# zenithfang/supervised_dispnet

Hardware: AMD Instinct MI355X
Metric: images/sec fwd+bwd Disp_vgg_BN 128x416 b32 @1/2/4/8 GPU (higher is better)
Workload: dtype f32 (Winograd forward / input gradient / weight gradient form each f32 product from three exact bf16 pieces per operand on the bf16 matrix cores, six partial products, f32 accumulate; error vs fp64 at or below the f32 matrix instruction's)

## Files before the change

### include/dispnet_hip.h

```cpp
#ifndef DISPNET_HIP_H_
#define DISPNET_HIP_H_

#include <stddef.h>
#include <stdint.h>

#ifdef __cplusplus
extern "C" {
#endif

typedef void* dn_stream_t;

enum dn_status {
  DN_OK = 0,
  DN_ERR_BAD_ARG = -1,
  DN_ERR_UNSUPPORTED = -2,
  DN_ERR_WORKSPACE = -3,
  DN_ERR_LAUNCH = -4
};

void dn_reload_knobs(void);
int dn_version(void);
const char* dn_last_error(void);
const char* dn_last_kernel(void);
int dn_device_arch_ok(void);
// ... 14 lines not shown
  DN_CONVT_FWD = 2,
  DN_CONVT_DGRAD = 3
};

typedef struct dn_operand {
  const float* data;
  int32_t C;
  int32_t up_shift;
  int64_t stride_n, stride_h, stride_w, stride_c;
  const float* scale;
  const float* shift;
} dn_operand;

typedef struct dn_result {
  float* data;
  int32_t C;
  int32_t accumulate;
  int64_t stride_n, stride_h, stride_w;
} dn_result;

typedef struct dn_conv_desc {
  int32_t kind;
  int32_t N;
  int32_t IH, IW;
  int32_t OH, OW;
  int32_t R, S, stride, pad;
  int32_t n_in;
  dn_operand in[DN_MAX_OPERANDS];
  int32_t n_out;
  dn_result out[DN_MAX_OPERANDS];
  const float* w_packed;
  const float* bias;
  int32_t act;
  float act_p0, act_p1;
  float* bn_partial;
  int32_t pad_mode;
  int32_t compute;
  int32_t dilation;
  const float* bnb_y;
  const float* bnb_scale;
  const float* bnb_shift;
  const float* bnb_mean;
  const float* bnb_invstd;
  float* bnb_partial;
  void* splitk_ws;
  int64_t splitk_ws_bytes;
  float* recip_out;
  const float* bnf_gamma;
  const float* bnf_beta;
  float* bnf_running_mean;
  float* bnf_running_var;
  int64_t* bnf_num_batches_tracked;
  float bnf_momentum, bnf_eps;
  float* bnf_mean;
  float* bnf_invstd;
  float* bnf_scale;
  float* bnf_shift;
  float* bnb_dgamma;
  float* bnb_dbeta;
} dn_conv_desc;

enum { DN_COMPUTE_DEFAULT = 0, DN_COMPUTE_BF16 = 1, DN_COMPUTE_F32X3 = 2, DN_COMPUTE_F32 = 3 };

int64_t dn_conv_packed_weight_elems(const dn_conv_desc* d);
int dn_conv_pack_weights(const dn_conv_desc* d, const float* w, float* w_packed, dn_stream_t stream);
int64_t dn_pack_entry_bytes(void);
int dn_pack_entry_fill(const dn_conv_desc* d, const float* w, float* w_packed, void* entry_host);
int dn_pack_many(const void* entries_dev, int32_t n_direct, int32_t n_wino, int32_t n_wino_bf16, int32_t n_wino_x3, dn_stream_t stream);
int32_t dn_conv_weight_layout(const dn_conv_desc* d);
int32_t dn_conv_bn_partial_rows(const dn_conv_desc* d);
int64_t dn_conv_splitk_workspace_bytes(const dn_conv_desc* d);
int32_t dn_conv_fwd_folds_bn_finalize(const dn_conv_desc* d);
int32_t dn_conv_dgrad_folds_bn_sums(const dn_conv_desc* d);
int32_t dn_conv_dgrad_fuses_bn_sums(const dn_conv_desc* d);
int32_t dn_conv_fwd_fuses_reciprocal(const dn_conv_desc* d);
int dn_conv2d_fwd(const dn_conv_desc* d, dn_stream_t stream);
int dn_conv2d_dgrad(const dn_conv_desc* d, dn_stream_t stream);
int dn_convT2d_fwd(const dn_conv_desc* d, dn_stream_t stream);
int dn_convT2d_dgrad(const dn_conv_desc* d, dn_stream_t stream);

size_t dn_conv_wgrad_workspace_bytes(const dn_conv_desc* fwd);
int dn_conv2d_wgrad(const dn_conv_desc* fwd, const float* dy, float* dw, void* workspace, size_t workspace_bytes,
                    dn_stream_t stream);

int dn_bn_finalize(const float* partial, int32_t rows, int32_t C, int64_t count, const float* conv_bias,
                   const float* gamma, const float* beta, float* running_mean, float* running_var, float momentum,
                   float eps, float* mean, float* invstd, float* scale, float* shift, int64_t* num_batches_tracked,
                   dn_stream_t stream);
int dn_bn_eval_affine(int32_t C, const float* gamma, const float* beta, const float* running_mean,
                      const float* running_var, float eps, float* scale, float* shift, dn_stream_t stream);
int dn_bn_relu_pool_fwd(const float* y, const float* scale, const float* shift, int32_t N, int32_t H, int32_t W,
                        int32_t C, float* pooled, uint8_t* idx, dn_stream_t stream);
int dn_bn_relu_pool_bwd(const float* dpooled, const uint8_t* idx, const float* y, const float* mean,
                        const float* invstd, int32_t N, int32_t H, int32_t W, int32_t C, float* dz, float* partial,
                        dn_stream_t stream);
int dn_maxpool2_bwd(const float* dpooled, const uint8_t* idx, int32_t N, int32_t H, int32_t W, int32_t C, float* dx, int32_t accumulate,
                    dn_stream_t stream);
int dn_bn_relu_bwd_reduce(float* da_dz, const float* y, const float* scale, const float* shift, const float* mean,
                          const float* invstd, int64_t rows, int32_t C, float* partial, dn_stream_t stream);
int dn_bn_bwd_apply(float* dz_dy, const float* y, const float* mean, const float* invstd, const float* gamma,
                    const float* partial, int32_t partial_rows, int32_t partial_stride, int32_t partial_offset, int64_t rows,
                    int32_t C, float* dgamma, float* dbeta, dn_stream_t stream);
int dn_bn_relu_bwd_sums(const float* da, const float* y, const float* scale, const float* shift, const float* mean, const float* invstd,
                        int64_t rows, int32_t C, float* partial, dn_stream_t stream);
int dn_bn_relu_pool_bwd_sums(const float* dpooled, const uint8_t* idx, const float* y, const float* mean, const float* invstd, int32_t N,
                             int32_t H, int32_t W, int32_t C, float* partial, dn_stream_t stream);
int dn_bn_bwd_apply_relu(float* da_dy, const float* y, const float* scale, const float* shift, const float* mean, const float* invstd,
                         const float* gamma, const float* partial, int32_t partial_rows, int32_t partial_stride, int32_t partial_offset,
                         int64_t rows, int32_t C, float* dgamma, float* dbeta, dn_stream_t stream);
int dn_bn_bwd_apply_pool(const float* dpooled, const uint8_t* idx, const float* y, const float* mean, const float* invstd, const float* gamma,
                         const float* partial, int32_t partial_rows, int32_t partial_stride, int32_t partial_offset, int32_t N, int32_t H,
                         int32_t W, int32_t C, float* dy, float* dgamma, float* dbeta, dn_stream_t stream);
int32_t dn_reduce_blocks(int64_t rows, int32_t C);

int dn_act_bwd_reduce_from(const float* g_in, float* g_out, const float* y_post, int32_t act, float p0, float p1, int64_t rows, int32_t C,
                           float* partial, dn_stream_t stream);
int dn_act_bwd_reduce(float* g, const float* y_post, int32_t act, float p0, float p1, int64_t rows, int32_t C,
                      float* partial, dn_stream_t stream);
int dn_colsum_finalize(const float* partial, int32_t rows, int32_t C, int32_t stride, int32_t offset, float* out,
                       dn_stream_t stream);
int dn_upsample2x_nearest_bwd(const float* dfull, int32_t N, int32_t h, int32_t w, float* dlow, int32_t accumulate,
                              dn_stream_t stream);
int dn_upsample2x_nearest_bwd_nhwc(const float* dfull, int32_t N, int32_t h, int32_t w, int32_t C, float* dlow, int32_t accumulate,
                                   dn_stream_t stream);
int dn_reflect_fold(const float* dxp, int32_t N, int32_t H, int32_t W, int32_t C, int32_t pad, float* dx, int32_t accumulate,
                    dn_stream_t stream);
int dn_bn_add_relu_fwd(const float* y, const float* scale, const float* shift, const float* r, const float* r_scale, const float* r_shift,
                       int64_t rows, int32_t C, float* out, dn_stream_t stream);
int dn_bn_add_relu_bwd(const float* gout, const float* out, const float* y, const float* mean, const float* invstd, const float* r,
                       const float* r_mean, const float* r_invstd, int64_t rows, int32_t C, float* dz_y, float* dr, int32_t dr_accumulate,
                       float* partial, dn_stream_t stream);
int32_t dn_maxpool3s2_out(int32_t H, int32_t ceil_mode);
int dn_maxpool3s2_fwd(const float* x, int32_t N, int32_t H, int32_t W, int32_t C, int32_t ceil_mode, float* out, uint8_t* idx, dn_stream_t stream);
int dn_maxpool3s2_bwd(const float* dout, const uint8_t* idx, int32_t N, int32_t H, int32_t W, int32_t C, int32_t ceil_mode, float* dx,
                      int32_t accumulate, dn_stream_t stream);
int dn_sub_div(const float* x, int64_t n, float sub, float div, float* out, dn_stream_t stream);
int dn_upsample2x_bilinear_fwd(const float* low, int32_t N, int32_t h, int32_t w, int32_t OH, int32_t OW, float* out,
                               dn_stream_t stream);
int dn_upsample2x_bilinear_bwd(const float* dout, int32_t N, int32_t h, int32_t w, int32_t OH, int32_t OW, float* dlow,
                               int32_t accumulate, dn_stream_t stream);
int32_t dn_bn_stats_rows(int64_t rows);
int dn_bn_stats_partial(const float* x, int64_t rows, int32_t C, float* partial, dn_stream_t stream);
int dn_bn_apply_fwd(const float* y, const float* scale, const float* shift, int64_t rows, int32_t C, float* out, dn_stream_t stream);
int dn_phase_bias_add(float* x, int32_t N, int32_t H2, int32_t W2, int32_t C, const float* bias4, dn_stream_t stream);
size_t dn_phase_colsum_workspace_bytes(int32_t C);
int dn_phase_colsum(const float* g, int32_t N, int32_t H, int32_t W, int32_t C, float* workspace, float* out4, dn_stream_t stream);
int dn_act_fwd(const float* x, int64_t n, int32_t act, float p0, float p1, float* out, dn_stream_t stream);
int dn_resize_bilinear_fwd(const float* in, int32_t N, int32_t IH, int32_t IW, int32_t OH, int32_t OW, int32_t align_corners, float* out,
                           dn_stream_t stream);
int dn_resize_bilinear_bwd(const float* dout, int32_t N, int32_t IH, int32_t IW, int32_t OH, int32_t OW, int32_t align_corners, float* din,
                           int32_t accumulate, dn_stream_t stream);
int dn_spatial_mean_fwd(const float* x, int32_t N, int64_t HW, int32_t C, float scale, float* out, dn_stream_t stream);
int dn_spatial_mean_bwd(const float* dout, int32_t N, int64_t HW, int32_t C, float scale, float* dx, dn_stream_t stream);
int dn_reciprocal_fwd(const float* x, float* y, int64_t n, dn_stream_t stream);
int dn_reciprocal_bwd(const float* dy, const float* y, float* dx, int64_t n, dn_stream_t stream);

enum dn_masked_loss_kind { DN_LOSS_L1 = 0, DN_LOSS_L2 = 1, DN_LOSS_BERHU = 2, DN_LOSS_SCALE_INV = 3 };
#define DN_LOSS_STATS 8
size_t dn_masked_loss_workspace_bytes(int32_t G, int64_t pixels);
int dn_masked_loss_fwd(const float* gt, const float* pred, int32_t G, int64_t pixels, float max_depth, int32_t kind, float weight,
                       int32_t accumulate, float* stats, void* workspace, size_t workspace_bytes, float* loss, dn_stream_t stream);
int dn_masked_loss_fwd_fused(const float* gt, const float* pred, int32_t G, int64_t pixels, float max_depth, int32_t kind, float weight,
                             int32_t accumulate, float* stats, void* workspace, size_t workspace_bytes, float* loss, int32_t* counter,
                             dn_stream_t stream);
int dn_masked_loss_stats(const float* gt, const float* pred, int32_t G, int64_t pixels, float max_depth, int32_t kind, int32_t pass,
                         float* stats, void* workspace, size_t workspace_bytes, dn_stream_t stream);
int dn_masked_loss_finalize(float* stats, int32_t G, int32_t kind, float weight, int32_t accumulate, float* loss, dn_stream_t stream);
int dn_masked_loss_bwd(const float* gt, const float* pred, const float* stats, const float* dloss, int32_t G, int64_t pixels,
                       float max_depth, int32_t kind, float weight, float* dpred, dn_stream_t stream);
int dn_pyramid_down2(const float* in, int32_t N, int32_t H, int32_t W, int32_t mode, float* out, dn_stream_t stream);
int dn_upsample_int_fwd(const float* low, int32_t N, int32_t h, int32_t w, int32_t scale, int32_t mode, float* out, dn_stream_t stream);
int dn_upsample_int_bwd(const float* dout, int32_t N, int32_t h, int32_t w, int32_t scale, int32_t mode, float* dlow, dn_stream_t stream);
int32_t dn_reduce1d_blocks(int64_t n);
int dn_explainability_fwd(const float* mask, int64_t n, float weight, int32_t accumulate, float* partial, float* loss, dn_stream_t stream);
int dn_explainability_bwd(const float* mask, const float* dloss, int64_t n, float* dmask, dn_stream_t stream);
int32_t dn_smooth_blocks(int32_t B, int32_t H, int32_t W);
int dn_smooth2_fwd(const float* map, int32_t B, int32_t H, int32_t W, float weight, float* partial, float* loss,
                   dn_stream_t stream);
int dn_smooth2_bwd(const float* map, const float* dloss, int32_t B, int32_t H, int32_t W, float weight, float* dmap,
                   dn_stream_t stream);
int dn_compute_errors(const float* gt, const float* pred, int32_t B, int32_t H, int32_t W, float max_depth, int32_t y1,
                      int32_t y2, int32_t x1, int32_t x2, int32_t median_scaling, float* scratch, float* out8,
                      dn_stream_t stream);

int dn_pose_proj_fwd(const float* pose, int64_t pose_stride_b, const float* K, const float* Kinv, int32_t B, int32_t rotation_mode,
                     float downscale, float* proj, float* kinv_scaled, dn_stream_t stream);
int32_t dn_warp_blocks(int32_t h, int32_t w);
int dn_pose_proj_bwd(const float* pose, int64_t pose_stride_b, const float* K, int32_t B, int32_t rotation_mode, float downscale,
                     const float* dproj_partial, int32_t nblk, float* dpose, int64_t dpose_stride_b, int32_t accumulate,
                     dn_stream_t stream);
int dn_inverse_warp_fwd(const float* img, const float* depth, const float* proj, const float* kinv, int32_t B, int32_t h, int32_t w,
                        int32_t padding_mode, int32_t align_corners, float* warped, dn_stream_t stream);
// ... 108 lines not shown
```

### supervised_dispnet_amd/_lib.py

```python
import ctypes as C
import os
import pathlib

_PKG = pathlib.Path(__file__).resolve().parent
LIB_PATH = pathlib.Path(os.environ.get("DISPNET_HIP_LIB", _PKG / "libdispnet_hip.so"))

EXPECTED_ABI = 21

DN_MAX_OPERANDS = 3
ACT_NONE, ACT_RELU, ACT_LEAKY, ACT_ELU, ACT_SIGMOID_AFFINE = 0, 1, 2, 3, 4
COMPUTE_DEFAULT, COMPUTE_BF16, COMPUTE_F32X3, COMPUTE_F32 = 0, 1, 2, 3
CONV_FWD, CONV_DGRAD, CONVT_FWD, CONVT_DGRAD = 0, 1, 2, 3
LOSS_L1, LOSS_L2, LOSS_BERHU, LOSS_SCALE_INV = 0, 1, 2, 3
LOSS_STATS = 8

_f32p = C.c_void_p


class Operand(C.Structure):
    _fields_ = [("data", _f32p), ("C", C.c_int32), ("up_shift", C.c_int32),
                ("stride_n", C.c_int64), ("stride_h", C.c_int64), ("stride_w", C.c_int64), ("stride_c", C.c_int64),
                ("scale", _f32p), ("shift", _f32p)]


class Result(C.Structure):
    _fields_ = [("data", _f32p), ("C", C.c_int32), ("accumulate", C.c_int32),
                ("stride_n", C.c_int64), ("stride_h", C.c_int64), ("stride_w", C.c_int64)]


class ConvDesc(C.Structure):
    _fields_ = [("kind", C.c_int32), ("N", C.c_int32), ("IH", C.c_int32), ("IW", C.c_int32), ("OH", C.c_int32),
                ("OW", C.c_int32), ("R", C.c_int32), ("S", C.c_int32), ("stride", C.c_int32), ("pad", C.c_int32),
                ("n_in", C.c_int32), ("in_", Operand * DN_MAX_OPERANDS),
                ("n_out", C.c_int32), ("out", Result * DN_MAX_OPERANDS),
                ("w_packed", _f32p), ("bias", _f32p), ("act", C.c_int32), ("act_p0", C.c_float), ("act_p1", C.c_float),
                ("bn_partial", _f32p), ("pad_mode", C.c_int32), ("compute", C.c_int32), ("dilation", C.c_int32),
                ("bnb_y", _f32p), ("bnb_scale", _f32p), ("bnb_shift", _f32p), ("bnb_mean", _f32p), ("bnb_invstd", _f32p), ("bnb_partial", _f32p),
                ("splitk_ws", _f32p), ("splitk_ws_bytes", C.c_int64), ("recip_out", _f32p),
                ("bnf_gamma", _f32p), ("bnf_beta", _f32p), ("bnf_running_mean", _f32p), ("bnf_running_var", _f32p),
                ("bnf_num_batches_tracked", C.c_void_p), ("bnf_momentum", C.c_float), ("bnf_eps", C.c_float),
                ("bnf_mean", _f32p), ("bnf_invstd", _f32p), ("bnf_scale", _f32p), ("bnf_shift", _f32p),
                ("bnb_dgamma", _f32p), ("bnb_dbeta", _f32p)]


_P = C.POINTER
_i32, _i64, _f, _d, _vp, _sz = C.c_int32, C.c_int64, C.c_float, C.c_double, C.c_void_p, C.c_size_t

SIGNATURES = {
    "dn_version": (C.c_int, []),
    "dn_reload_knobs": (None, []),
    "dn_last_error": (C.c_char_p, []),
    "dn_last_kernel": (C.c_char_p, []),
    "dn_device_arch_ok": (C.c_int, []),
    "dn_conv_packed_weight_elems": (_i64, [_P(ConvDesc)]),
    "dn_conv_pack_weights": (C.c_int, [_P(ConvDesc), _vp, _vp, _vp]),
    "dn_pack_entry_bytes": (_i64, []),
    "dn_pack_entry_fill": (C.c_int, [_P(ConvDesc), _vp, _vp, _vp]),
    "dn_pack_many": (C.c_int, [_vp, _i32, _i32, _i32, _i32, _vp]),
    "dn_conv_weight_layout": (_i32, [_P(ConvDesc)]),
    "dn_conv_bn_partial_rows": (_i32, [_P(ConvDesc)]),
    "dn_conv_dgrad_fuses_bn_sums": (_i32, [_P(ConvDesc)]),
    "dn_conv_fwd_fuses_reciprocal": (_i32, [_P(ConvDesc)]),
    "dn_conv_splitk_workspace_bytes": (_i64, [_P(ConvDesc)]),
    "dn_conv_fwd_folds_bn_finalize": (_i32, [_P(ConvDesc)]),
    "dn_conv_dgrad_folds_bn_sums": (_i32, [_P(ConvDesc)]),
    "dn_conv2d_fwd": (C.c_int, [_P(ConvDesc), _vp]),
    "dn_conv2d_dgrad": (C.c_int, [_P(ConvDesc), _vp]),
    "dn_convT2d_fwd": (C.c_int, [_P(ConvDesc), _vp]),
    "dn_convT2d_dgrad": (C.c_int, [_P(ConvDesc), _vp]),
    "dn_conv_wgrad_workspace_bytes": (_sz, [_P(ConvDesc)]),
    "dn_conv2d_wgrad": (C.c_int, [_P(ConvDesc), _vp, _vp, _vp, _sz, _vp]),
    "dn_bn_finalize": (C.c_int, [_vp, _i32, _i32, _i64, _vp, _vp, _vp, _vp, _vp, _f, _f, _vp, _vp, _vp, _vp, _vp, _vp]),
    "dn_bn_eval_affine": (C.c_int, [_i32, _vp, _vp, _vp, _vp, _f, _vp, _vp, _vp]),
    "dn_bn_relu_pool_fwd": (C.c_int, [_vp, _vp, _vp, _i32, _i32, _i32, _i32, _vp, _vp, _vp]),
    "dn_bn_relu_bwd_sums": (C.c_int, [_vp, _vp, _vp, _vp, _vp, _vp, _i64, _i32, _vp, _vp]),
    "dn_bn_relu_pool_bwd_sums": (C.c_int, [_vp, _vp, _vp, _vp, _vp, _i32, _i32, _i32, _i32, _vp, _vp]),
    "dn_bn_bwd_apply_relu": (C.c_int, [_vp, _vp, _vp, _vp, _vp, _vp, _vp, _vp, _i32, _i32, _i32, _i64, _i32, _vp, _vp, _vp]),
    "dn_bn_bwd_apply_pool": (C.c_int, [_vp, _vp, _vp, _vp, _vp, _vp, _vp, _i32, _i32, _i32, _i32, _i32, _i32, _i32, _vp, _vp, _vp, _vp]),
    "dn_maxpool2_bwd": (C.c_int, [_vp, _vp, _i32, _i32, _i32, _i32, _vp, _i32, _vp]),
    "dn_bn_relu_pool_bwd": (C.c_int, [_vp, _vp, _vp, _vp, _vp, _i32, _i32, _i32, _i32, _vp, _vp, _vp]),
    "dn_bn_relu_bwd_reduce": (C.c_int, [_vp, _vp, _vp, _vp, _vp, _vp, _i64, _i32, _vp, _vp]),
    "dn_bn_bwd_apply": (C.c_int, [_vp, _vp, _vp, _vp, _vp, _vp, _i32, _i32, _i32, _i64, _i32, _vp, _vp, _vp]),
    "dn_reduce_blocks": (_i32, [_i64, _i32]),
    "dn_act_bwd_reduce": (C.c_int, [_vp, _vp, _i32, _f, _f, _i64, _i32, _vp, _vp]),
    "dn_act_bwd_reduce_from": (C.c_int, [_vp, _vp, _vp, _i32, _f, _f, _i64, _i32, _vp, _vp]),
    "dn_colsum_finalize": (C.c_int, [_vp, _i32, _i32, _i32, _i32, _vp, _vp]),
    "dn_upsample2x_nearest_bwd": (C.c_int, [_vp, _i32, _i32, _i32, _vp, _i32, _vp]),
    "dn_upsample2x_nearest_bwd_nhwc": (C.c_int, [_vp, _i32, _i32, _i32, _i32, _vp, _i32, _vp]),
    "dn_reflect_fold": (C.c_int, [_vp, _i32, _i32, _i32, _i32, _i32, _vp, _i32, _vp]),
    "dn_bn_add_relu_fwd": (C.c_int, [_vp, _vp, _vp, _vp, _vp, _vp, _i64, _i32, _vp, _vp]),
    "dn_bn_add_relu_bwd": (C.c_int, [_vp, _vp, _vp, _vp, _vp, _vp, _vp, _vp, _i64, _i32, _vp, _vp, _i32, _vp, _vp]),
    "dn_maxpool3s2_out": (_i32, [_i32, _i32]),
    "dn_maxpool3s2_fwd": (C.c_int, [_vp, _i32, _i32, _i32, _i32, _i32, _vp, _vp, _vp]),
    "dn_maxpool3s2_bwd": (C.c_int, [_vp, _vp, _i32, _i32, _i32, _i32, _i32, _vp, _i32, _vp]),
    "dn_bn_stats_rows": (_i32, [_i64]),
    "dn_bn_stats_partial": (C.c_int, [_vp, _i64, _i32, _vp, _vp]),
    "dn_bn_apply_fwd": (C.c_int, [_vp, _vp, _vp, _i64, _i32, _vp, _vp]),
    "dn_act_fwd": (C.c_int, [_vp, _i64, _i32, _f, _f, _vp, _vp]),
    "dn_phase_bias_add": (C.c_int, [_vp, _i32, _i32, _i32, _i32, _vp, _vp]),
    "dn_phase_colsum_workspace_bytes": (_sz, [_i32]),
    "dn_phase_colsum": (C.c_int, [_vp, _i32, _i32, _i32, _i32, _vp, _vp, _vp]),
    "dn_resize_bilinear_fwd": (C.c_int, [_vp, _i32, _i32, _i32, _i32, _i32, _i32, _vp, _vp]),
    "dn_resize_bilinear_bwd": (C.c_int, [_vp, _i32, _i32, _i32, _i32, _i32, _i32, _vp, _i32, _vp]),
    "dn_sub_div": (C.c_int, [_vp, _i64, _f, _f, _vp, _vp]),
    "dn_spatial_mean_fwd": (C.c_int, [_vp, _i32, _i64, _i32, _f, _vp, _vp]),
    "dn_spatial_mean_bwd": (C.c_int, [_vp, _i32, _i64, _i32, _f, _vp, _vp]),
    "dn_upsample2x_bilinear_fwd": (C.c_int, [_vp, _i32, _i32, _i32, _i32, _i32, _vp, _vp]),
    "dn_upsample2x_bilinear_bwd": (C.c_int, [_vp, _i32, _i32, _i32, _i32, _i32, _vp, _i32, _vp]),
    "dn_reciprocal_fwd": (C.c_int, [_vp, _vp, _i64, _vp]),
    "dn_reciprocal_bwd": (C.c_int, [_vp, _vp, _vp, _i64, _vp]),
    "dn_masked_loss_workspace_bytes": (_sz, [_i32, _i64]),
    "dn_masked_loss_fwd": (C.c_int, [_vp, _vp, _i32, _i64, _f, _i32, _f, _i32, _vp, _vp, _sz, _vp, _vp]),
    "dn_masked_loss_fwd_fused": (C.c_int, [_vp, _vp, _i32, _i64, _f, _i32, _f, _i32, _vp, _vp, _sz, _vp, _vp, _vp]),
    "dn_masked_loss_stats": (C.c_int, [_vp, _vp, _i32, _i64, _f, _i32, _i32, _vp, _vp, _sz, _vp]),
    "dn_masked_loss_finalize": (C.c_int, [_vp, _i32, _i32, _f, _i32, _vp, _vp]),
    "dn_masked_loss_bwd": (C.c_int, [_vp, _vp, _vp, _vp, _i32, _i64, _f, _i32, _f, _vp, _vp]),
    "dn_pyramid_down2": (C.c_int, [_vp, _i32, _i32, _i32, _i32, _vp, _vp]),
    "dn_upsample_int_fwd": (C.c_int, [_vp, _i32, _i32, _i32, _i32, _i32, _vp, _vp]),
    "dn_upsample_int_bwd": (C.c_int, [_vp, _i32, _i32, _i32, _i32, _i32, _vp, _vp]),
    "dn_reduce1d_blocks": (_i32, [_i64]),
    "dn_explainability_fwd": (C.c_int, [_vp, _i64, _f, _i32, _vp, _vp, _vp]),
    "dn_explainability_bwd": (C.c_int, [_vp, _vp, _i64, _vp, _vp]),
    "dn_smooth_blocks": (_i32, [_i32, _i32, _i32]),
    "dn_smooth2_fwd": (C.c_int, [_vp, _i32, _i32, _i32, _f, _vp, _vp, _vp]),
    "dn_smooth2_bwd": (C.c_int, [_vp, _vp, _i32, _i32, _i32, _f, _vp, _vp]),
    "dn_compute_errors": (C.c_int, [_vp, _vp, _i32, _i32, _i32, _f, _i32, _i32, _i32, _i32, _i32, _vp, _vp, _vp]),
    "dn_pose_proj_fwd": (C.c_int, [_vp, _i64, _vp, _vp, _i32, _i32, _f, _vp, _vp, _vp]),
    "dn_warp_blocks": (_i32, [_i32, _i32]),
    "dn_pose_proj_bwd": (C.c_int, [_vp, _i64, _vp, _i32, _i32, _f, _vp, _i32, _vp, _i64, _i32, _vp]),
    "dn_inverse_warp_fwd": (C.c_int, [_vp, _vp, _vp, _vp, _i32, _i32, _i32, _i32, _i32, _vp, _vp]),
    "dn_inverse_warp_bwd": (C.c_int, [_vp, _vp, _vp, _vp, _i32, _i32, _i32, _i32, _i32, _vp, _vp, _i32, _vp, _vp]),
    "dn_photometric_fwd": (C.c_int, [_vp, _vp, _vp, _vp, _vp, _vp, _i64, _i32, _i32, _i32, _i32, _i32, _f, _i32, _vp, _vp, _vp]),
    "dn_photometric_bwd": (C.c_int, [_vp, _vp, _vp, _vp, _vp, _vp, _i64, _i32, _i32, _i32, _i32, _i32, _f, _vp, _vp, _i32, _vp, _vp,
                                     _i64, _vp]),
    "dn_area_down": (C.c_int, [_vp, _i64, _i32, _i32, _i32, _vp, _vp]),
    "dn_ssim_fwd": (C.c_int, [_vp, _vp, _i64, _i32, _i32, _vp, _vp]),
    "dn_ssim_bwd": (C.c_int, [_vp, _vp, _vp, _i64, _i32, _i32, _vp, _vp, _vp, _vp]),
    "dn_edge_smooth_blocks": (_i32, [_i32, _i32, _i32]),
    "dn_edge_smooth_fwd": (C.c_int, [_vp, _vp, _i32, _i32, _i32, _i32, _vp, _vp, _vp]),
    "dn_edge_smooth_bwd": (C.c_int, [_vp, _vp, _vp, _i32, _i32, _i32, _i32, _vp, _vp]),
    "dn_ordinal_fwd": (C.c_int, [_vp, _i64, _i64, _i64, _i32, _i64, _i32, _vp, _vp, _vp]),
    "dn_ordinal_bwd": (C.c_int, [_vp, _i64, _i64, _i64, _vp, _vp, _i32, _i64, _i32, _vp, _vp]),
    "dn_ordinal_loss_blocks": (_i32, [_i32, _i64]),
    "dn_ordinal_loss_fwd": (C.c_int, [_vp, _vp, _vp, _i32, _i64, _i32, _f, _vp, _vp, _vp, _vp]),
    "dn_ordinal_loss_finalize": (C.c_int, [_vp, _vp, _vp]),
    "dn_ordinal_loss_bwd": (C.c_int, [_vp, _vp, _vp, _vp, _vp, _i32, _i64, _i32, _f, _f, _vp, _vp]),
    "dn_ord_head_supported": (_i32, [_i32, _i64, _i32]),
    "dn_ord_head_bwd_blocks": (_i32, [_i32, _i64]),
    "dn_ord_head_fwd": (C.c_int, [_vp, _vp, _vp, _vp, _i32, _i64, _i32, _vp, _vp, _vp]),
    "dn_ord_head_bwd": (C.c_int, [_vp, _vp, _vp, _vp, _vp, _i32, _i64, _i32, _vp, _i32, _vp, _vp, _vp, _vp]),
    "dn_sid_labels": (C.c_int, [_vp, _i64, _f, _f, _vp, _vp]),
    "dn_sid_depth": (C.c_int, [_vp, _i64, _f, _f, _vp, _vp]),
    "dn_channel_scale": (C.c_int, [_vp, _vp, _i32, _i64, _i32, _vp, _vp]),
    "dn_adam_step": (C.c_int, [_vp, _vp, _vp, _vp, _i64, _d, _d, _d, _d, _d, _i32, _d, _vp]),
    "dn_adam_step_dev": (C.c_int, [_vp, _vp, _vp, _vp, _i64, _vp, _d, _d, _vp, _vp, _d, _vp]),
    "dn_adam_tick": (C.c_int, [_vp, _vp, _vp, _vp]),
    "dn_fill": (C.c_int, [_vp, _f, _i64, _vp]),
    "dn_copy": (C.c_int, [_vp, _vp, _i64, _vp]),
    "dn_tape_begin": (_vp, []),
    "dn_tape_end": (C.c_int, [_vp]),
# ... 89 lines not shown
```

### supervised_dispnet_amd/csrc/dn_conv.hip

```cpp
#include <atomic>
#include <stdlib.h>
#include <type_traits>
#include <utility>

#include "dn_device.h"

namespace dn {

constexpr int LDK = 36;

struct AGroup {
  f32x4 v;
  bool ok;
};

__device__ __forceinline__ AGroup gather4(const KOperand& S, int kl, int ntaps, const int* taps, int n, int by, int bx,
                                          bool rowvalid, int IH, int IW, int j_vec, int c_vec, int reflect) {
  AGroup r;
  r.v = f32x4{0.f, 0.f, 0.f, 0.f};
  r.ok = false;
  if (S.vec) {
    if (rowvalid && j_vec < ntaps) {
      int t = taps[j_vec];
      int iy = by + (int)(short)(t & 0xffff), ix = bx + (t >> 16);
// ... 2165 lines not shown
    }
  }
  if (rc != DN_OK) return rc;
  return launch_wgrad_reduce(p, dw, s);
}

static bool wgrad_split_plans(const dn_conv_desc* fwd, dn_conv_desc* d1, dn_conv_desc* d2, IgemmParams* p1, IgemmParams* p2, size_t* w1,
                              size_t* w2) {
  if (fwd->kind != DN_CONV_FWD || fwd->n_in < 2 || fwd->in[fwd->n_in - 1].C != 1) return false;
  *d1 = *fwd;
  d1->n_in = fwd->n_in - 1;
  *d2 = *fwd;
  d2->n_in = 1;
  d2->in[0] = fwd->in[fwd->n_in - 1];
  if (build_plan(d1, true, p1) != DN_OK || build_plan(d2, true, p2) != DN_OK) return false;
  int cin_total = 0;
  for (int i = 0; i < fwd->n_in; ++i) cin_total += fwd->in[i].C;
  if (wino_wgrad_eligible(d1, *p1)) {
    p1->dw_cin_total = cin_total;
    *w1 = (wino_wgrad_workspace_bytes(*p1) + 255) / 256 * 256;
  } else {
    return false;
  }
  p2->in[0].ch_off = cin_total - 1;
  p2->D1 = cin_total;
  choose_splits(p2);
  *w2 = generic_wgrad_workspace_bytes(*p2);
  return true;
}

static int tap_windows(const IgemmParams& p) {
  const int nt = p.ph[0].ntaps;
  if (nt <= 32 || p.reflect || p.nphases != 1 || knobs().no_tap_windows) return 1;
  return (nt + 31) / 32;
}

static void tap_window_plan(const IgemmParams& full, int w, int nw, IgemmParams* q) {
  *q = full;
  const int nt = full.ph[0].ntaps, per = (nt + nw - 1) / nw;
  const int t0 = w * per, t1 = t0 + per < nt ? t0 + per : nt;
  for (int t = t0; t < t1; ++t) {
    q->tdy[t - t0] = full.tdy[full.ph[0].tap0 + t];
    q->tdx[t - t0] = full.tdx[full.ph[0].tap0 + t];
    q->tr[t - t0] = full.tr[full.ph[0].tap0 + t];
    q->ts[t - t0] = full.ts[full.ph[0].tap0 + t];
  }
  q->ph[0].tap0 = 0;
  q->ph[0].ntaps = t1 - t0;
  int nch = 0;
  for (int i = 0; i < q->n_in; ++i) nch += (q->ph[0].ntaps * q->in[i].C + kChunk - 1) / kChunk;
  q->ph[0].nchunks = nch;
  q->uni32 = 1;
  q->wg_uniform = 1;
  for (int i = 0; i < q->n_in; ++i) {
    const KOperand& o = q->in[i];
    if (!o.small) q->uni32 = 0;
    if (!o.small || (!o.vec && o.scale != nullptr) || o.C >= 32768) q->wg_uniform = 0;
  }
}

struct WgradFamily {
  const char* name;
  bool (*eligible)(const dn_conv_desc* fwd, const IgemmParams& p);
  size_t (*workspace_bytes)(const dn_conv_desc* fwd, const IgemmParams& p);
  bool dy_aligned16;
  bool (*switched_off)();
  int (*launch)(const dn_conv_desc* fwd, IgemmParams& p, float* dw, hipStream_t s);
};
static const WgradFamily kWgradFamilies[] = {
    {"head", head_wgrad_eligible, [](const dn_conv_desc*, const IgemmParams& p) { return head_wgrad_workspace_bytes(p); }, false,
     [] { return knobs().no_direct; },
     [](const dn_conv_desc*, IgemmParams& p, float* dw, hipStream_t s) { return launch_head_wgrad(p, dw, p.ws, s); }},
    {"winograd", wino_wgrad_eligible, [](const dn_conv_desc*, const IgemmParams& p) { return wino_wgrad_workspace_bytes(p); }, false, nullptr,
     [](const dn_conv_desc*, IgemmParams& p, float* dw, hipStream_t s) { return launch_wino_wgrad(p, dw, s); }},
    {"lds3", lds3_wgrad_eligible, [](const dn_conv_desc*, const IgemmParams& p) { return lds3_wgrad_workspace_bytes(p); }, true, nullptr,
     launch_lds3_wgrad},
    {"lds3k", lds3k_wgrad_eligible, [](const dn_conv_desc*, const IgemmParams& p) { return lds3k_wgrad_workspace_bytes(p); }, true, nullptr,
     launch_lds3k_wgrad},
    {"stemk", stemk_wgrad_eligible, stemk_wgrad_workspace_bytes, true, nullptr, launch_stemk_wgrad},
    {"thin", thin_wgrad_eligible, [](const dn_conv_desc*, const IgemmParams& p) { return thin_wgrad_workspace_bytes(p); }, false, nullptr,
     [](const dn_conv_desc*, IgemmParams& p, float* dw, hipStream_t s) { return launch_thin_wgrad(p, dw, s); }},
};

extern "C" {

int64_t dn_pack_entry_bytes(void) { return (int64_t)sizeof(PackEntry); }

int dn_pack_entry_fill(const dn_conv_desc* d, const float* w, float* w_packed, void* entry_host) {
  DN_REQUIRE(d && w && w_packed && entry_host, DN_ERR_BAD_ARG, "dn_pack_entry_fill: null pointer");
  PackEntry* e = reinterpret_cast<PackEntry*>(entry_host);
  int rc = build_plan(d, false, &e->p);
  if (rc != DN_OK) return rc;
  e->w = w;
  e->wp = w_packed;
  const ConvFamily* f = conv_route(d, e->p);
  e->wino = f->weight_layout ? f->weight_layout(e->p) : 0;
  if (e->wino) {
    e->total = wino_packed_elems(e->p);
    e->NS = ((e->p.Ntot + 63) / 64 * 64) / 32;
  } else {
    e->total = direct_packed_elems(e->p);
    e->NS = 0;
  }
  return e->wino;
}

int dn_pack_many(const void* entries_dev, int32_t n_direct, int32_t n_wino, int32_t n_wino16, int32_t n_wino_x3, dn_stream_t stream) {
  DN_REQUIRE(entries_dev && n_direct >= 0 && n_wino >= 0 && n_wino16 >= 0 && n_wino_x3 >= 0, DN_ERR_BAD_ARG, "dn_pack_many: bad argument");
  const PackEntry* tab = reinterpret_cast<const PackEntry*>(entries_dev);
  hipStream_t s = as_stream(stream);
  if (n_direct > 0) {
    DN_LAUNCH(pack_weights_many_kernel, dim3(knobs().pack_blocks, n_direct), dim3(256), 0, s, tab);
    int rc = check_launch("pack_weights_many_kernel");
    if (rc != DN_OK) return rc;
  }
  if (n_wino > 0) {
    int rc = launch_wino_pack_many(tab, n_direct, n_wino, s);
    if (rc != DN_OK) return rc;
  }
  if (n_wino16 > 0) {
    int rc = launch_wino_pack16_many(tab, n_direct + n_wino, n_wino16, 1, s);
    if (rc != DN_OK) return rc;
  }
  if (n_wino_x3 > 0) return launch_wino_pack16_many(tab, n_direct + n_wino + n_wino16, n_wino_x3, 3, s);
  return DN_OK;
}

int dn_conv_pack_weights(const dn_conv_desc* d, const float* w, float* w_packed, dn_stream_t stream) {
  IgemmParams p;
  int rc = build_plan(d, false, &p);
  if (rc != DN_OK) return rc;
  DN_REQUIRE(w != nullptr && w_packed != nullptr, DN_ERR_BAD_ARG, "null weight pointer");
  const ConvFamily* f = conv_route(d, p);
  if (const int wl = f->weight_layout ? f->weight_layout(p) : 0)
    return wl == 1 ? launch_wino_pack(p, w, w_packed, as_stream(stream)) : launch_wino_pack16(p, w, w_packed, wl == 3 ? 3 : 1, as_stream(stream));
  const long long total = direct_packed_elems(p);
  if (total == 0) return DN_OK;
  int blocks = (int)((total + 255) / 256);
  if (blocks > 4096) blocks = 4096;
  DN_LAUNCH(pack_weights_kernel, dim3(blocks), dim3(256), 0, as_stream(stream), p, w, w_packed, total);
  return check_launch("pack_weights_kernel");
}

int dn_conv2d_fwd(const dn_conv_desc* d, dn_stream_t stream) { return run_conv(d, DN_CONV_FWD, stream); }
int dn_conv2d_dgrad(const dn_conv_desc* d, dn_stream_t stream) { return run_conv(d, DN_CONV_DGRAD, stream); }
int dn_convT2d_fwd(const dn_conv_desc* d, dn_stream_t stream) { return run_conv(d, DN_CONVT_FWD, stream); }
int dn_convT2d_dgrad(const dn_conv_desc* d, dn_stream_t stream) { return run_conv(d, DN_CONVT_DGRAD, stream); }

size_t dn_conv_wgrad_workspace_bytes(const dn_conv_desc* fwd) {
  IgemmParams p;
  if (build_plan(fwd, true, &p) != DN_OK) return 0;
  choose_splits(&p);
  size_t need = generic_wgrad_workspace_bytes(p);
  for (const WgradFamily& f : kWgradFamilies)
    if (f.eligible(fwd, p) && f.workspace_bytes(fwd, p) > need) need = f.workspace_bytes(fwd, p);
  {
    dn_conv_desc d1, d2;
    IgemmParams p1, p2;
    size_t w1 = 0, w2 = 0;
    if (wgrad_split_plans(fwd, &d1, &d2, &p1, &p2, &w1, &w2) && w1 + w2 > need) need = w1 + w2;
  }
  const int nw = tap_windows(p);
  for (int w = 0; w < nw && nw > 1; ++w) {
    IgemmParams q;
    tap_window_plan(p, w, nw, &q);
    choose_splits(&q);
    if (generic_wgrad_workspace_bytes(q) > need) need = generic_wgrad_workspace_bytes(q);
  }
  return need;
}

int dn_conv2d_wgrad(const dn_conv_desc* fwd, const float* dy, float* dw, void* workspace, size_t workspace_bytes,
                    dn_stream_t stream) {
  IgemmParams p;
  int rc = build_plan(fwd, true, &p);
  if (rc != DN_OK) return rc;
  DN_REQUIRE(dy != nullptr && dw != nullptr && workspace != nullptr, DN_ERR_BAD_ARG, "null pointer");
  const hipStream_t s = as_stream(stream);
  for (const WgradFamily& f : kWgradFamilies) {
    if (!f.eligible(fwd, p) || (f.switched_off && f.switched_off()) || workspace_bytes < f.workspace_bytes(fwd, p)) continue;
    if (f.dy_aligned16 && (reinterpret_cast<uintptr_t>(dy) & 15) != 0) continue;
    for (int i = 0; i < p.n_in; ++i) DN_REQUIRE(p.in[i].p != nullptr, DN_ERR_BAD_ARG, "operand %d has no data", i);
    p.g = dy;
    p.ws = reinterpret_cast<float*>(workspace);
    return f.launch(fwd, p, dw, s);
  }
  {
    dn_conv_desc d1, d2;
    IgemmParams p1, p2;
    size_t w1 = 0, w2 = 0;
    if (wgrad_split_plans(fwd, &d1, &d2, &p1, &p2, &w1, &w2) && workspace_bytes >= w1 + w2) {
      for (int i = 0; i < fwd->n_in; ++i) DN_REQUIRE(fwd->in[i].data != nullptr, DN_ERR_BAD_ARG, "operand %d has no data", i);
      if (wino_wgrad_eligible(&d1, p1)) {
        p1.g = dy;
        p1.ws = reinterpret_cast<float*>(workspace);
        rc = launch_wino_wgrad(p1, dw, s);
      } else {
        rc = generic_wgrad(&d1, p1, dy, dw, workspace, w1, s);
      }
      if (rc != DN_OK) return rc;
      return generic_wgrad(&d2, p2, dy, dw, reinterpret_cast<char*>(workspace) + w1, w2, s);
    }
  }
  if (const int nw = tap_windows(p); nw > 1 && fwd->kind == DN_CONV_FWD) {
    for (int w = 0; w < nw; ++w) {
      IgemmParams q;
      tap_window_plan(p, w, nw, &q);
      rc = generic_wgrad(fwd, q, dy, dw, workspace, workspace_bytes, s);
      if (rc != DN_OK) return rc;
    }
    return DN_OK;
  }
  return generic_wgrad(fwd, p, dy, dw, workspace, workspace_bytes, s);
}

}
```

### supervised_dispnet_amd/csrc/dn_device.h

```cpp
#pragma once
#include <type_traits>
#include <utility>

#include "dn_internal.h"

namespace dn {

typedef float f32x2 __attribute__((ext_vector_type(2)));
typedef float f32x4 __attribute__((ext_vector_type(4)));
typedef float f32x16 __attribute__((ext_vector_type(16)));
typedef __bf16 bf16x2 __attribute__((ext_vector_type(2)));
typedef __bf16 bf16x4 __attribute__((ext_vector_type(4)));
typedef __bf16 bf16x8 __attribute__((ext_vector_type(8)));
typedef int i32x2 __attribute__((ext_vector_type(2)));
typedef int i32x4 __attribute__((ext_vector_type(4)));
typedef unsigned u32x4 __attribute__((ext_vector_type(4)));

template <class F, int... I>
__device__ __forceinline__ void static_for_impl(F&& f, std::integer_sequence<int, I...>) {
  (f(std::integral_constant<int, I>{}), ...);
}
template <int N, class F>
__device__ __forceinline__ void static_for(F&& f) {
  static_for_impl(f, std::make_integer_sequence<int, N>{});
}

__device__ __forceinline__ float apply_act(float v, int act, float p0, float p1) {
  switch (act) {
    case DN_ACT_RELU: return v > 0.f ? v : 0.f;
    case DN_ACT_LEAKY: return v > 0.f ? v : v * p0;
    case DN_ACT_ELU: return v > 0.f ? v : (expf(v) - 1.f);
    case DN_ACT_SIGMOID_AFFINE: return p0 / (1.f + expf(-v)) + p1;
    default: return v;
  }
}

__device__ __forceinline__ f32x4 apply_act4(f32x4 v, int act, float p0, float p1) {
  f32x4 r = v;
  switch (act) {
    case DN_ACT_RELU:
#pragma unroll
      for (int e = 0; e < 4; ++e) r[e] = v[e] > 0.f ? v[e] : 0.f;
      break;
    case DN_ACT_LEAKY:
#pragma unroll
      for (int e = 0; e < 4; ++e) r[e] = v[e] > 0.f ? v[e] : v[e] * p0;
      break;
    case DN_ACT_ELU:
#pragma unroll
      for (int e = 0; e < 4; ++e) r[e] = v[e] > 0.f ? v[e] : (expf(v[e]) - 1.f);
      break;
    case DN_ACT_SIGMOID_AFFINE:
#pragma unroll
      for (int e = 0; e < 4; ++e) r[e] = p0 / (1.f + expf(-v[e])) + p1;
      break;
    default: break;
  }
  return r;
}

__device__ __forceinline__ void split3(const float (&v)[8], bf16x8& h, bf16x8& m, bf16x8& l) {
#pragma unroll
  for (int e = 0; e < 8; e += 2) {
    const f32x2 x = f32x2{v[e], v[e + 1]};
    const bf16x2 h2 = __builtin_convertvector(x, bf16x2);
    const f32x2 r = x - __builtin_convertvector(h2, f32x2);
    const bf16x2 m2 = __builtin_convertvector(r, bf16x2);
    const f32x2 q = r - __builtin_convertvector(m2, f32x2);
    const bf16x2 l2 = __builtin_convertvector(q, bf16x2);
    h[e] = h2[0]; h[e + 1] = h2[1];
    m[e] = m2[0]; m[e + 1] = m2[1];
    l[e] = l2[0]; l[e + 1] = l2[1];
  }
}

__device__ __forceinline__ void wino_split3(float x, __bf16* pc) {
  pc[0] = (__bf16)x;
  const float r1 = x - (float)pc[0];
  pc[1] = (__bf16)r1;
  pc[2] = (__bf16)(r1 - (float)pc[1]);
}

__device__ __forceinline__ float wave_sum(float v) {
#pragma unroll
  for (int o = 32; o > 0; o >>= 1) v += __shfl_xor(v, o);
  return v;
}

template <int ROT>
__device__ __forceinline__ float dpp_row_ror(float v) {
  return __builtin_bit_cast(float, __builtin_amdgcn_update_dpp(0, __builtin_bit_cast(int, v), 0x120 + ROT, 0xf, 0xf, false));
}
__device__ __forceinline__ float row16_sum(float v) {
  v += dpp_row_ror<8>(v);
  v += dpp_row_ror<4>(v);
  v += dpp_row_ror<2>(v);
  v += dpp_row_ror<1>(v);
  return v;
}

template <int VW> struct VecOf;
template <> struct VecOf<4> { typedef f32x4 type; };
template <> struct VecOf<2> { typedef f32x2 type; };

template <int VW>
__device__ __forceinline__ typename VecOf<VW>::type buffer_load_vec(__amdgpu_buffer_rsrc_t r, int voffset) {
  if constexpr (VW == 4) {
    const i32x4 v = __builtin_amdgcn_raw_buffer_load_b128(r, voffset, 0, 0);
    return __builtin_bit_cast(f32x4, v);
  } else {
    const i32x2 v = __builtin_amdgcn_raw_buffer_load_b64(r, voffset, 0, 0);
    return __builtin_bit_cast(f32x2, v);
  }
}

__device__ __forceinline__ unsigned fastdiv_dev(unsigned n, unsigned d, unsigned M, unsigned* rem) {
  unsigned q = __umulhi(n, M);
  unsigned r = n - q * d;
  const bool fix = r >= d;
  q += fix ? 1u : 0u;
  r -= fix ? d : 0u;
  *rem = r;
  return q;
}

__device__ __forceinline__ int reflect_idx(int v, int n) {
  const int m = n - 1;
  int a = v < 0 ? -v : v;
  a = m - a;
  a = a < 0 ? -a : a;
  return m - a;
}

__device__ __forceinline__ int select_operand(const IgemmParams& p, int ntaps, int kc, int* kc_local) {
  int s = 0;
#pragma unroll
  for (int i = 0; i < DN_MAX_OPERANDS - 1; ++i) {
    if (s == i && i < p.n_in - 1) {
      int nch = (ntaps * p.in[i].C + kChunk - 1) / kChunk;
      if (kc >= nch) {
        kc -= nch;
// ... 10 lines not shown
```

### supervised_dispnet_amd/csrc/dn_internal.h

```cpp
#pragma once
#include <hip/hip_runtime.h>
#include <hip/hip_ext.h>
#include <stdint.h>
#include <stdio.h>

#include <atomic>
#include <functional>
#include <tuple>
#include <type_traits>

#include "dispnet_hip.h"

namespace dn {

void set_error(const char* fmt, ...);
void set_last_kernel(const char* fmt, ...);
int check_launch(const char* what);

static inline hipStream_t as_stream(dn_stream_t s) { return reinterpret_cast<hipStream_t>(s); }

struct LaunchTape;
extern std::atomic<LaunchTape*> g_tape_rec;
void tape_push(LaunchTape* t, std::function<void(hipEvent_t)>&& op, const void* kernel, hipStream_t stream);

// ... 141 lines not shown
  float* recip_out;
  float* ks_ws;
  size_t ks_ws_bytes;
  int T, TH, TW;
  unsigned mTW, mTH;
  BnFinalizeArgs bnf;
  float *bnb_dgamma, *bnb_dbeta;
  int* fold_cnt;
  int fold_bn, fold_bnb;
  int nmajor;
};

static inline unsigned fastdiv_magic(unsigned d) { return d <= 1 ? 0xFFFFFFFFu : (unsigned)(0x100000000ull / d); }

int build_plan(const dn_conv_desc* d, bool for_wgrad, IgemmParams* p);

inline long long direct_packed_elems(const IgemmParams& p) {
  const KPhase& last = p.ph[p.nphases - 1];
  return last.w_off + (long long)p.Npad * last.nchunks * kChunk;
}

struct PackEntry {
  IgemmParams p;
  const float* w;
  float* wp;
  long long total;
  int wino;
  int NS;
};
int launch_wino_pack_many(const PackEntry* tab_dev, int first, int n, hipStream_t stream);
int launch_wino_pack16_many(const PackEntry* tab_dev, int first, int n, int pieces, hipStream_t stream);
int launch_wino_pack16(const IgemmParams& p, const float* w, float* wp, int pieces, hipStream_t stream);
long long wino_packed_floats(const IgemmParams& p, int layout);
int wino_layout(const IgemmParams& p);

struct ConvFamily {
  const char* name;
  bool (*eligible)(const dn_conv_desc* d, const IgemmParams& p);
  bool (*switched_off)();
  int (*launch)(const dn_conv_desc* d, IgemmParams& p, hipStream_t s);
  int (*weight_layout)(const IgemmParams& p);
  size_t (*splitk_workspace_bytes)(const IgemmParams& p);
  bool (*fuses_reciprocal)(const IgemmParams& p);
  bool (*takes_bn_sums)(const dn_conv_desc* d);
  bool (*folds_bn_finalize)(IgemmParams& p);
  bool (*folds_bn_sums)(IgemmParams& p);
};
const ConvFamily* conv_route(const dn_conv_desc* d, const IgemmParams& p);

bool head_fwd_eligible(const dn_conv_desc* d, const IgemmParams& p);
int launch_head_fwd(const IgemmParams& p, hipStream_t stream);
bool head_fwd_fuses_reciprocal(const IgemmParams& p);
bool head_dgrad_eligible(const dn_conv_desc* d, const IgemmParams& p);
int launch_head_dgrad(const IgemmParams& p, hipStream_t stream);
bool head_wgrad_eligible(const dn_conv_desc* fwd, const IgemmParams& p);
size_t head_wgrad_workspace_bytes(const IgemmParams& p);
int launch_head_wgrad(const IgemmParams& p, float* dw, float* workspace, hipStream_t stream);

bool wino_eligible(const dn_conv_desc* d, const IgemmParams& p);
long long wino_packed_elems(const IgemmParams& p);
int launch_wino_pack(const IgemmParams& p, const float* w, float* wp, hipStream_t stream);
int launch_wino_conv(IgemmParams& p, hipStream_t stream);
void wino_prepare(IgemmParams& p);
bool wino_folds_bn_finalize(const IgemmParams& p);
bool wino_folds_bn_sums(const IgemmParams& p);
int wino_splitk_choice(const IgemmParams& p);
size_t conv_x3_splitk_workspace_upper_bytes(const IgemmParams& p);
size_t wino_splitk_workspace_bytes(const IgemmParams& p);
bool wino_wgrad_eligible(const dn_conv_desc* fwd, const IgemmParams& p);
size_t wino_wgrad_workspace_bytes(const IgemmParams& p);
int launch_wino_wgrad(IgemmParams& p, float* dw, hipStream_t stream);

bool thin_wgrad_eligible(const dn_conv_desc* fwd, const IgemmParams& p);
size_t thin_wgrad_workspace_bytes(const IgemmParams& p);
int launch_thin_wgrad(IgemmParams& p, float* dw, hipStream_t stream);
bool thin_conv_eligible(const dn_conv_desc* d, const IgemmParams& p);
int launch_thin_conv(const IgemmParams& p, hipStream_t stream);

bool lds3_conv_eligible(const dn_conv_desc* d, const IgemmParams& p);
int launch_lds3_conv(const dn_conv_desc* d, const IgemmParams& p, hipStream_t stream);
bool lds3_wgrad_eligible(const dn_conv_desc* fwd, const IgemmParams& p);
size_t lds3_wgrad_workspace_bytes(const IgemmParams& p);
int launch_lds3_wgrad(const dn_conv_desc* fwd, IgemmParams& p, float* dw, hipStream_t stream);
bool lds3k_wgrad_eligible(const dn_conv_desc* fwd, const IgemmParams& p);
size_t lds3k_wgrad_workspace_bytes(const IgemmParams& p);
int launch_lds3k_wgrad(const dn_conv_desc* fwd, IgemmParams& p, float* dw, hipStream_t stream);
int launch_wgrad_reduce(const IgemmParams& p, float* dw, hipStream_t stream);
bool wgrad_x3_eligible(const IgemmParams& p);
int launch_wgrad_x3(const IgemmParams& p, hipStream_t stream);
bool lds3k_conv_eligible(const dn_conv_desc* d, const IgemmParams& p);
int launch_lds3k_conv(const dn_conv_desc* d, const IgemmParams& p, hipStream_t stream);
bool stem3_conv_eligible(const dn_conv_desc* d, const IgemmParams& p);
bool stemk_conv_eligible(const dn_conv_desc* d, const IgemmParams& p);
int launch_stemk_conv(const dn_conv_desc* d, const IgemmParams& p, hipStream_t stream);
bool stemk_wgrad_eligible(const dn_conv_desc* d, const IgemmParams& p);
size_t stemk_wgrad_workspace_bytes(const dn_conv_desc* d, const IgemmParams& p);
int launch_stemk_wgrad(const dn_conv_desc* d, IgemmParams& p, float* dw, hipStream_t stream);
int launch_stem3_conv(const IgemmParams& p, hipStream_t stream);

}
```

### supervised_dispnet_amd/csrc/dn_lds3_wgrad.hip

```cpp
#include <stdlib.h>

#include "dn_device.h"

namespace dn {

struct WgGeo {
  int tilesX, tilesY, ntiles, per_xcd;
  long long slab;
  int dbgmode;
  long long* dbg;
};

constexpr int WG_TH = 8, WG_TW = 32;
constexpr int WG_GSTR = 528;
constexpr int WG_GPIECE = 16 * WG_GSTR;
constexpr int WG_XROWB = 96;
constexpr int WG_XSTR = 10 * WG_XROWB + 16;
constexpr int WG_XPIECE = 16 * WG_XSTR;
constexpr int WG_DCOLS = 36;
constexpr int WG16_LDS = 3 * WG_GPIECE + 3 * WG_XPIECE + 10 * WG_DCOLS * 4;

template <bool HAS1, bool DBG = false>
__global__ void __launch_bounds__(256, 2) lds3_wgrad16_kernel(const IgemmParams p, const WgGeo geo) {
  extern __shared__ __align__(16) char lds[];
// ... 116 lines not shown
      const int r = 2 * wave + rr;
      bf16x8 a[3];
#pragma unroll
      for (int P = 0; P < 3; ++P) a[P] = *reinterpret_cast<const bf16x8*>(Gp + P * WG_GPIECE + j * WG_GSTR + (r * 32 + 8 * g) * 2);
#pragma unroll
      for (int ty = 0; ty < 3; ++ty) {
        const char* rowb = Xp + j * WG_XSTR + (r + ty) * WG_XROWB + (8 * g + 8) * 2;
        u32x4 c[3];
        unsigned lf[3], rt[3];
#pragma unroll
        for (int P = 0; P < 3; ++P) {
          c[P] = *reinterpret_cast<const u32x4*>(rowb + P * WG_XPIECE);
          lf[P] = *reinterpret_cast<const unsigned*>(rowb + P * WG_XPIECE - 4);
          rt[P] = *reinterpret_cast<const unsigned*>(rowb + P * WG_XPIECE + 16);
        }
        bf16x8 bm[3], bz[3], bp[3];
#pragma unroll
        for (int P = 0; P < 3; ++P) {
          const u32x4 m4 = u32x4{__builtin_amdgcn_alignbit(c[P][0], lf[P], 16), __builtin_amdgcn_alignbit(c[P][1], c[P][0], 16),
                                 __builtin_amdgcn_alignbit(c[P][2], c[P][1], 16), __builtin_amdgcn_alignbit(c[P][3], c[P][2], 16)};
          const u32x4 p4 = u32x4{__builtin_amdgcn_alignbit(c[P][1], c[P][0], 16), __builtin_amdgcn_alignbit(c[P][2], c[P][1], 16),
                                 __builtin_amdgcn_alignbit(c[P][3], c[P][2], 16), __builtin_amdgcn_alignbit(rt[P], c[P][3], 16)};
          bm[P] = __builtin_bit_cast(bf16x8, m4);
          bz[P] = __builtin_bit_cast(bf16x8, c[P]);
          bp[P] = __builtin_bit_cast(bf16x8, p4);
        }
#pragma unroll
        for (int q = 0; q < 6; ++q) {
          acc[3 * ty + 0] = __builtin_amdgcn_mfma_f32_16x16x32_bf16(a[AS[q]], bm[BS[q]], acc[3 * ty + 0], 0, 0, 0);
          acc[3 * ty + 1] = __builtin_amdgcn_mfma_f32_16x16x32_bf16(a[AS[q]], bz[BS[q]], acc[3 * ty + 1], 0, 0, 0);
          acc[3 * ty + 2] = __builtin_amdgcn_mfma_f32_16x16x32_bf16(a[AS[q]], bp[BS[q]], acc[3 * ty + 2], 0, 0, 0);
        }
      }
      if constexpr (HAS1) {
        float v[8];
#pragma unroll
        for (int e = 0; e < 8; ++e) {
          const float x = Dp[r * WG_DCOLS + 8 * g + e + doff];
          v[e] = j < 9 ? x : 0.f;
        }
        bf16x8 b[3];
        split3(v, b[0], b[1], b[2]);
#pragma unroll
        for (int q = 0; q < 6; ++q) acc[9] = __builtin_amdgcn_mfma_f32_16x16x32_bf16(a[AS[q]], b[BS[q]], acc[9], 0, 0, 0);
      }
    }
    stamp(4);
    __syncthreads();
    stamp(5);
  }
  if constexpr (DBG) {
    if (lane == 0) {
      long long* o = geo.dbg + ((size_t)blockIdx.x * 8 + wave) * 8;
      for (int k = 0; k < 6; ++k) o[k] = tk[k];
      o[6] = (band_hi - band_lo - local + nlocal - 1) / nlocal;
    }
  }

  f32x4* red = reinterpret_cast<f32x4*>(lds);
#pragma unroll
  for (int t = 0; t < NT; ++t) red[(wave * NT + t) * 64 + lane] = acc[t];
  __syncthreads();
  const int Kp = p.ph[0].nchunks * kChunk;
  const int kbase1 = ((9 * 16 + kChunk - 1) / kChunk) * kChunk;
  float* slab = p.ws + (long long)blockIdx.x * geo.slab;
  for (int it = tid; it < NT * 64; it += 256) {
    const int t = it >> 6, l = it & 63;
    const f32x4 s = (red[(0 * NT + t) * 64 + l] + red[(1 * NT + t) * 64 + l]) + (red[(2 * NT + t) * 64 + l] + red[(3 * NT + t) * 64 + l]);
    const int jj = l & 15, gg = l >> 4;
    const int k = t < 9 ? t * 16 + jj : kbase1 + jj;
    if (t < 9 || jj < 9) {
#pragma unroll
      for (int e = 0; e < 4; ++e) slab[(long long)(4 * gg + e) * Kp + k] = s[e];
    }
  }
}

constexpr int WS_GSTR = 272;
constexpr int WS_GPIECE = 64 * WS_GSTR;
constexpr int WS_ICOLS = 36;
constexpr int WS_IPLANE = 10 * WS_ICOLS;
constexpr int WGS_LDS = 3 * WS_GPIECE + 3 * WS_IPLANE * 4;

__global__ void __launch_bounds__(256, 2) lds3_wgrad_stem_kernel(const IgemmParams p, const WgGeo geo) {
  extern __shared__ __align__(16) char lds[];
  char* Gp = lds;
  float* Ip = reinterpret_cast<float*>(lds + 3 * WS_GPIECE);
  const int tid = threadIdx.x, lane = tid & 63, wave = tid >> 6;
  const int j = lane & 15, g = lane >> 4;
  const KOperand& S = p.in[0];
  const int C = S.C, K = 9 * C;
  const __amdgpu_buffer_rsrc_t rg = __builtin_amdgcn_make_buffer_rsrc(const_cast<float*>(p.g), 0, 0x80000000u, 0x00020000);
  const __amdgpu_buffer_rsrc_t rx = __builtin_amdgcn_make_buffer_rsrc(const_cast<float*>(S.p), 0, 0x80000000u, 0x00020000);

  f32x4 acc[4][2];
#pragma unroll
  for (int m = 0; m < 4; ++m)
#pragma unroll
    for (int nt = 0; nt < 2; ++nt) acc[m][nt] = f32x4{0.f, 0.f, 0.f, 0.f};
  int ioff[2];
  bool ilive[2];
#pragma unroll
  for (int nt = 0; nt < 2; ++nt) {
    const int col = 16 * nt + j;
    ilive[nt] = col < K;
    const int tap = ilive[nt] ? col / C : 0, ci = ilive[nt] ? col - tap * C : 0;
    ioff[nt] = ci * WS_IPLANE + (tap / 3) * WS_ICOLS + (tap % 3);
  }

  f32x4 vg[8];
  float vi[4];
  auto issue_g = [&](int t, int h) __attribute__((always_inline)) {
    const int txb = t % geo.tilesX, q1 = t / geo.tilesX;
    const int tyb = q1 % geo.tilesY, n = q1 / geo.tilesY;
    const int pxg = tid & 15, cq = tid >> 4, row = pxg >> 2, cgp = pxg & 3;
    const int gy = tyb * WG_TH + 4 * h + row;
#pragma unroll
    for (int i = 0; i < 8; ++i) {
      const int gx = txb * WG_TW + 8 * cgp + i;
      const bool ok = gy < p.GH && gx < p.GW;
      const int off = (((n * p.GH + gy) * p.GW + gx) * p.Ntot + 4 * cq) * 4;
      vg[i] = __builtin_bit_cast(f32x4, __builtin_amdgcn_raw_buffer_load_b128(rg, ok ? off : -1, 0, 0));
    }
  };
  auto issue_img = [&](int t) __attribute__((always_inline)) {
    const int txb = t % geo.tilesX, q1 = t / geo.tilesX;
    const int tyb = q1 % geo.tilesY, n = q1 / geo.tilesY;
#pragma unroll
    for (int r = 0; r < 4; ++r) {
      const int it = tid + 256 * r;
      const int c = it / 340, px = it - c * 340;
      const int row = px / 34, col = px - row * 34;
      const int iy = tyb * WG_TH - 1 + row, ix = txb * WG_TW - 1 + col;
      const bool ok = c < C && (unsigned)iy < (unsigned)p.IH && (unsigned)ix < (unsigned)p.IW;
      const int off = (n * (int)S.sn + iy * (int)S.sh + ix * (int)S.sw + c * (int)S.sc) * 4;
      vi[r] = __builtin_bit_cast(float, __builtin_amdgcn_raw_buffer_load_b32(rx, ok ? off : -1, 0, 0));
    }
  };
  auto store_g = [&]() __attribute__((always_inline)) {
    const int pxg = tid & 15, cq = tid >> 4;
#pragma unroll
    for (int e = 0; e < 4; ++e) {
      const float v[8] = {vg[0][e], vg[1][e], vg[2][e], vg[3][e], vg[4][e], vg[5][e], vg[6][e], vg[7][e]};
      bf16x8 h, m, l;
      split3(v, h, m, l);
      char* dst = Gp + (4 * cq + e) * WS_GSTR + pxg * 16;
      *reinterpret_cast<bf16x8*>(dst) = h;
      *reinterpret_cast<bf16x8*>(dst + WS_GPIECE) = m;
      *reinterpret_cast<bf16x8*>(dst + 2 * WS_GPIECE) = l;
    }
  };
  auto store_img = [&]() __attribute__((always_inline)) {
#pragma unroll
    for (int r = 0; r < 4; ++r) {
      const int it = tid + 256 * r;
      const int c = it / 340, px = it - c * 340;
      const int row = px / 34, col = px - row * 34;
      if (c < 3) Ip[c * WS_IPLANE + row * WS_ICOLS + col] = vi[r];
    }
  };

  const int xcd = (int)blockIdx.x & 7, local = (int)blockIdx.x >> 3, nlocal = (int)gridDim.x >> 3;
  const int band_lo = xcd * geo.per_xcd, band_hi = min(band_lo + geo.per_xcd, geo.ntiles);
  constexpr int AS[6] = {0, 0, 1, 0, 1, 2}, BS[6] = {2, 1, 1, 0, 0, 0};
  if (band_lo + local < band_hi) {
    issue_g(band_lo + local, 0);
    issue_img(band_lo + local);
  }
  for (int t = band_lo + local; t < band_hi; t += nlocal) {
#pragma unroll 1
    for (int h = 0; h < 2; ++h) {
      store_g();
      if (h == 0) store_img();
      __syncthreads();
      if (h == 0) issue_g(t, 1);
      else if (t + nlocal < band_hi) {
        issue_g(t + nlocal, 0);
        issue_img(t + nlocal);
      }
      const int r = 4 * h + wave;
      bf16x8 b[2][3];
#pragma unroll
      for (int nt = 0; nt < 2; ++nt) {
        float v[8];
#pragma unroll
        for (int e = 0; e < 8; ++e) {
          const float x = Ip[r * WS_ICOLS + 8 * g + e + ioff[nt]];
          v[e] = ilive[nt] ? x : 0.f;
        }
        split3(v, b[nt][0], b[nt][1], b[nt][2]);
      }
#pragma unroll
      for (int m = 0; m < 4; ++m) {
        bf16x8 a[3];
#pragma unroll
        for (int P = 0; P < 3; ++P) a[P] = *reinterpret_cast<const bf16x8*>(Gp + P * WS_GPIECE + (16 * m + j) * WS_GSTR + (wave * 32 + 8 * g) * 2);
#pragma unroll
        for (int q = 0; q < 6; ++q)
#pragma unroll
          for (int nt = 0; nt < 2; ++nt) acc[m][nt] = __builtin_amdgcn_mfma_f32_16x16x32_bf16(a[AS[q]], b[nt][BS[q]], acc[m][nt], 0, 0, 0);
      }
      __syncthreads();
    }
  }

  f32x4* red = reinterpret_cast<f32x4*>(lds);
#pragma unroll
  for (int m = 0; m < 4; ++m)
#pragma unroll
    for (int nt = 0; nt < 2; ++nt) red[((wave * 4 + m) * 2 + nt) * 64 + lane] = acc[m][nt];
  __syncthreads();
  const int Kp = p.ph[0].nchunks * kChunk;
  float* slab = p.ws + (long long)blockIdx.x * geo.slab;
  for (int it = tid; it < 8 * 64; it += 256) {
    const int mn = it >> 6, l = it & 63, m = mn >> 1, nt = mn & 1;
    const f32x4 s = (red[((0 * 4 + m) * 2 + nt) * 64 + l] + red[((1 * 4 + m) * 2 + nt) * 64 + l]) +
                    (red[((2 * 4 + m) * 2 + nt) * 64 + l] + red[((3 * 4 + m) * 2 + nt) * 64 + l]);
    const int jj = l & 15, gg = l >> 4, k = 16 * nt + jj;
    if (k < K) {
#pragma unroll
      for (int e = 0; e < 4; ++e) slab[(long long)(16 * m + 4 * gg + e) * Kp + k] = s[e];
    }
  }
}

static int lds3_wgrad_form(const dn_conv_desc* d, const IgemmParams& p) {
  if (knobs().no_lds3 || norm_compute(d->compute) != DN_COMPUTE_F32X3) return 0;
  if (d->kind != DN_CONV_FWD || d->R != 3 || d->S != 3 || d->stride != 1 || d->pad != 1 || d->pad_mode != 0 || d->dilation > 1) return 0;
  if (d->IH != d->OH || d->IW != d->OW) return 0;
  if ((long long)p.M * p.Ntot * 4 + 64 >= (1ll << 31) || (reinterpret_cast<uintptr_t>(p.g) & 15)) return 0;
  for (int t = 0; t < 9; ++t)
    if (p.tdy[t] != t / 3 - 1 || p.tdx[t] != t % 3 - 1) return 0;
  const KOperand& a = p.in[0];
  if (!a.small || a.scale != nullptr || a.up != 0) return 0;
  if (p.Ntot == 16 && a.C == 16 && a.vec) {
    if (p.n_in == 1) return 1;
    const KOperand& b = p.in[1];
    if (p.n_in == 2 && b.C == 1 && b.small && b.scale == nullptr) return 2;
    return 0;
  }
  if (p.Ntot == 64 && p.n_in == 1 && a.C >= 1 && a.C <= 3) return 3;
  return 0;
}

static int lds3_wgrad_blocks(const IgemmParams& p) {
  const int ntiles = p.N * ((p.GH + WG_TH - 1) / WG_TH) * ((p.GW + WG_TW - 1) / WG_TW);
  int blocks = ntiles < 512 ? ntiles : 512;
  return (blocks + 7) / 8 * 8;
}

bool lds3_wgrad_eligible(const dn_conv_desc* d, const IgemmParams& p) { return lds3_wgrad_form(d, p) != 0; }

size_t lds3_wgrad_workspace_bytes(const IgemmParams& p) {
  return (size_t)lds3_wgrad_blocks(p) * p.Npad * p.ph[0].nchunks * kChunk * sizeof(float);
}

int launch_lds3_wgrad(const dn_conv_desc* d, IgemmParams& p, float* dw, hipStream_t stream) {
  const int form = lds3_wgrad_form(d, p);
  WgGeo geo;
  geo.tilesX = (p.GW + WG_TW - 1) / WG_TW;
  geo.tilesY = (p.GH + WG_TH - 1) / WG_TH;
  geo.ntiles = p.N * geo.tilesX * geo.tilesY;
  geo.per_xcd = (geo.ntiles + 7) / 8;
  geo.slab = (long long)p.Npad * p.ph[0].nchunks * kChunk;
  geo.dbg = knobs().lds3_dbg ? reinterpret_cast<long long*>(knobs().wino_dbgptr) : nullptr;
  geo.dbgmode = knobs().lds3_dbg;
  const int blocks = lds3_wgrad_blocks(p);
  hipError_t e = hipSuccess;
  if (geo.dbg != nullptr && form == 2) {
    e = hipFuncSetAttribute(reinterpret_cast<const void*>(lds3_wgrad16_kernel<true, true>), hipFuncAttributeMaxDynamicSharedMemorySize, WG16_LDS);
    if (e == hipSuccess) DN_LAUNCH((lds3_wgrad16_kernel<true, true>), dim3(blocks), dim3(256), (size_t)WG16_LDS, stream, p, geo);
    set_last_kernel("dn::lds3_wgrad16_kernel<true>");
  } else if (form == 3) {
    e = hipFuncSetAttribute(reinterpret_cast<const void*>(lds3_wgrad_stem_kernel), hipFuncAttributeMaxDynamicSharedMemorySize, WGS_LDS);
    if (e == hipSuccess) DN_LAUNCH(lds3_wgrad_stem_kernel, dim3(blocks), dim3(256), (size_t)WGS_LDS, stream, p, geo);
    set_last_kernel("dn::lds3_wgrad_stem_kernel");
  } else if (form == 2) {
    e = hipFuncSetAttribute(reinterpret_cast<const void*>(lds3_wgrad16_kernel<true>), hipFuncAttributeMaxDynamicSharedMemorySize, WG16_LDS);
    if (e == hipSuccess) DN_LAUNCH(lds3_wgrad16_kernel<true>, dim3(blocks), dim3(256), (size_t)WG16_LDS, stream, p, geo);
    set_last_kernel("dn::lds3_wgrad16_kernel<true>");
  } else if (form == 1) {
    e = hipFuncSetAttribute(reinterpret_cast<const void*>(lds3_wgrad16_kernel<false>), hipFuncAttributeMaxDynamicSharedMemorySize, WG16_LDS);
    if (e == hipSuccess) DN_LAUNCH(lds3_wgrad16_kernel<false>, dim3(blocks), dim3(256), (size_t)WG16_LDS, stream, p, geo);
    set_last_kernel("dn::lds3_wgrad16_kernel<false>");
  } else {
    set_error("launch_lds3_wgrad: no form");
    return DN_ERR_UNSUPPORTED;
  }
  if (e != hipSuccess) {
    set_error("lds3 wgrad: hipFuncSetAttribute: %s", hipGetErrorString(e));
    return DN_ERR_LAUNCH;
  }
  int rc = check_launch("lds3_wgrad_kernel");
  if (rc != DN_OK) return rc;
  p.splits = blocks;
  return launch_wgrad_reduce(p, dw, stream);
}

}

namespace dn {

constexpr int WK_TH = 2;
constexpr int WK_GSTR = WK_TH * 32 * 2 + 16;
constexpr int WK_GPIECE = 32 * WK_GSTR;
constexpr int WK_XROWS = WK_TH + 2;
constexpr int WK_XSTR = WK_XROWS * WG_XROWB + 16;
constexpr int WK_NCI = 96;
constexpr int WK_XPIECE = WK_NCI * WK_XSTR;
constexpr int WK_LDS = 3 * WK_GPIECE + 3 * WK_XPIECE + WK_XROWS * WG_DCOLS * 4;

template <bool HAS1, bool DBG = false>
__global__ void __launch_bounds__(512, 2) lds3k_wgrad_kernel(const IgemmParams p, const WgGeo geo, int c0) {
  extern __shared__ __align__(16) char lds[];
  char* Gp = lds;
  char* Xp = lds + 3 * WK_GPIECE;
  float* Dp = reinterpret_cast<float*>(lds + 3 * WK_GPIECE + 3 * WK_XPIECE);
  const int tid = threadIdx.x, lane = tid & 63, wave = tid >> 6;
  const int j = lane & 15, g = lane >> 4;
  const KOperand& S0 = p.in[0];
  const bool two = p.n_in - (HAS1 ? 1 : 0) == 2;
  const KOperand& S1 = p.in[two ? 1 : 0];
  const __amdgpu_buffer_rsrc_t rg = __builtin_amdgcn_make_buffer_rsrc(const_cast<float*>(p.g), 0, 0x80000000u, 0x00020000);
  const __amdgpu_buffer_rsrc_t r0 = __builtin_amdgcn_make_buffer_rsrc(const_cast<float*>(S0.p), 0, 0x80000000u, 0x00020000);
  const __amdgpu_buffer_rsrc_t r1 = __builtin_amdgcn_make_buffer_rsrc(const_cast<float*>(S1.p), 0, 0x80000000u, 0x00020000);
  const KOperand& SD = p.in[HAS1 ? p.n_in - 1 : 0];
  const __amdgpu_buffer_rsrc_t rd = __builtin_amdgcn_make_buffer_rsrc(const_cast<float*>(SD.p), 0, 0x80000000u, 0x00020000);

  const int nunits = wave < 2 ? 3 : 2;
  f32x4 acc[3][3][2];
#pragma unroll
  for (int u = 0; u < 3; ++u)
#pragma unroll
    for (int x = 0; x < 3; ++x)
#pragma unroll
      for (int m = 0; m < 2; ++m) acc[u][x][m] = f32x4{0.f, 0.f, 0.f, 0.f};
  f32x4 accd[2] = {f32x4{0.f, 0.f, 0.f, 0.f}, f32x4{0.f, 0.f, 0.f, 0.f}};
  const int dtap = j < 9 ? j : 0;
  const int doff = (dtap / 3) * WG_DCOLS + (dtap % 3);

  f32x4 va[8], vb[8];
  float dv = 0.f;
  const int nq0 = two ? c0 >> 2 : 24, n0jobs = 24 * nq0;
  auto decode = [&](int job, int& quad, int& rc, bool& second) __attribute__((always_inline)) {
    second = job >= n0jobs;
    const int jj = second ? job - n0jobs : job, nqh = (second ? 24 - nq0 : nq0) >> 2;
    const int rc_lo = jj & 3, q_lo = (jj >> 2) & 3, hi = jj >> 4;
    const int rc_hi = hi / nqh, q_hi = hi - rc_hi * nqh;
    rc = 4 * rc_hi + rc_lo;
    quad = (second ? nq0 : 0) + 4 * q_hi + q_lo;
  };
  int quadA, rcA, quadB, rcB;
  bool secA, secB;
  decode(tid, quadA, rcA, secA);
  decode(512 + (tid & 63), quadB, rcB, secB);
  const bool secAu = __builtin_amdgcn_readfirstlane((int)secA) != 0, secBu = __builtin_amdgcn_readfirstlane((int)secB) != 0;
  const int waveu = __builtin_amdgcn_readfirstlane(wave);
  const bool hasB = waveu == 2 || waveu == 3;
  const __amdgpu_buffer_rsrc_t rA = secAu ? r1 : r0;
// ... 312 lines not shown
```

### supervised_dispnet_amd/csrc/dn_plan.hip

```cpp
#include <stdarg.h>
#include <stdlib.h>
#include <string.h>

#include <atomic>
#include <mutex>

#include "dn_internal.h"

namespace dn {

static thread_local char g_err[512] = "";

void set_error(const char* fmt, ...) {
  va_list ap;
  va_start(ap, fmt);
  vsnprintf(g_err, sizeof(g_err), fmt, ap);
  va_end(ap);
}

static thread_local char g_kernel[160] = "";

void set_last_kernel(const char* fmt, ...) {
  va_list ap;
  va_start(ap, fmt);
// ... 272 lines not shown
          ph.ooy = py;
          ph.oox = px;
          for (int r = 0; r < d->R; ++r) {
            if (((py + pad - r * dil) % st + st) % st != 0) continue;
            for (int s = 0; s < d->S; ++s) {
              if (((px + pad - s * dil) % st + st) % st != 0) continue;
              DN_REQUIRE(nt < kMaxTaps, DN_ERR_UNSUPPORTED, "too many taps");
              p->tdy[nt] = (int8_t)floor_div(py + pad - r * dil, st);
              p->tdx[nt] = (int8_t)floor_div(px + pad - s * dil, st);
              p->tr[nt] = (int8_t)r;
              p->ts[nt] = (int8_t)s;
              ++nt;
            }
          }
          ph.ntaps = nt - ph.tap0;
        }
    }
    for (int i = 0; i < d->n_out; ++i) {
      KResult& r = p->out[i];
      r.p = d->out[i].data;
      r.C = d->out[i].C;
      r.accumulate = d->out[i].accumulate;
      r.sn = d->out[i].stride_n;
      r.sh = d->out[i].stride_h;
      r.sw = d->out[i].stride_w;
      r.n_begin = (i == 0) ? 0 : p->out[i - 1].n_begin + p->out[i - 1].C;
      r.linear = (p->nphases == 1 && r.sh == (long long)d->OW * r.sw && r.sn == (long long)d->OH * r.sh) ? 1 : 0;
    }
    DN_REQUIRE(d->bn_partial == nullptr || (d->n_out == 1 && p->nphases == 1), DN_ERR_UNSUPPORTED,
               "bn_partial needs a single un-phased result");
  }
  long long m = (long long)p->N * p->GH * p->GW;
  DN_REQUIRE(m > 0 && m < (1ll << 31), DN_ERR_UNSUPPORTED, "grid too large");
  p->M = (int)m;
  p->mGW = fastdiv_magic((unsigned)p->GW);
  p->mGH = fastdiv_magic((unsigned)p->GH);
  p->allvec = 1;
  p->uni32 = 1;
  p->any_affine = 0;
  for (int z = 0; z < p->nphases; ++z)
    if (p->ph[z].ntaps > 32) p->uni32 = 0;
  int n_fast = 0, n_uniform = 0;
  for (int i = 0; i < p->n_in; ++i) {
    const KOperand& o = p->in[i];
    if (o.scale != nullptr) p->any_affine = 1;
    p->in[i].small = offsets_fit_int32(p->in[i], p->N, p->IH, p->IW) && ((long long)p->N * (o.sn < 0 ? -o.sn : o.sn) + 16) * 4 < (1ll << 31) ? 1 : 0;
    if (!(p->in[i].vec && p->in[i].small)) p->allvec = 0;
    if (p->in[i].vec && p->in[i].small && o.up == 0 && (o.C % 32 == 0 || o.C == 4 || o.C == 8 || o.C == 16)) ++n_fast;
    if (p->in[i].vec && p->in[i].small && o.up == 0 && o.C % 32 == 0) ++n_uniform;
  }
  (void)n_fast;
  if (p->reflect) p->uni32 = 0;
  for (int i = 0; i < p->n_in; ++i)
    if (!p->in[i].small) p->uni32 = 0;
  p->wg_uniform = (!p->reflect && p->ph[0].ntaps <= 32) ? 1 : 0;
  for (int i = 0; i < p->n_in; ++i) {
    const KOperand& o = p->in[i];
    if (!o.small || (!o.vec && o.scale != nullptr) || o.C >= 32768) p->wg_uniform = 0;
  }
  (void)n_uniform;
  p->tile_store = false ? 0 : (false ? 1 : 2);
  p->compute = norm_compute(d->compute);
  p->BN = pick_bn(p->Ntot);
  p->Npad = ceil_div(p->Ntot, p->BN) * p->BN;
  long long woff = 0;
  for (int z = 0; z < p->nphases; ++z) {
    int nch = 0;
    for (int i = 0; i < p->n_in; ++i) nch += ceil_div(p->ph[z].ntaps * p->in[i].C, kChunk);
    p->ph[z].nchunks = nch;
    p->ph[z].w_off = woff;
    woff += (long long)p->Npad * nch * kChunk;
  }
  return DN_OK;
}

static const ConvFamily* plan_route(const dn_conv_desc* d, IgemmParams* p) {
  return build_plan(d, false, p) == DN_OK ? conv_route(d, *p) : nullptr;
}

}

extern "C" {

int dn_version(void) { return 21; }

void dn_reload_knobs(void) {
  std::lock_guard<std::mutex> lock(dn::g_knobs_mu);
  dn::read_knobs(&dn::g_knobs);
  dn::g_knobs_state.store(1, std::memory_order_release);
}

const char* dn_last_error(void) { return dn::g_err; }

const char* dn_last_kernel(void) { return dn::g_kernel; }

int dn_device_arch_ok(void) {
  int dev = 0;
  if (hipGetDevice(&dev) != hipSuccess) {
    dn::set_error("hipGetDevice failed (no HIP device?)");
    return DN_ERR_LAUNCH;
  }
  hipDeviceProp_t prop;
  if (hipGetDeviceProperties(&prop, dev) != hipSuccess) {
    dn::set_error("hipGetDeviceProperties failed");
    return DN_ERR_LAUNCH;
  }
  return strncmp(prop.gcnArchName, "gfx950", 6) == 0 ? 1 : 0;
}

int64_t dn_conv_packed_weight_elems(const dn_conv_desc* d) {
  dn::IgemmParams p;
  const dn::ConvFamily* f = dn::plan_route(d, &p);
  if (f == nullptr) return -1;
  return f->weight_layout ? dn::wino_packed_floats(p, f->weight_layout(p)) : dn::direct_packed_elems(p);
}

int32_t dn_conv_weight_layout(const dn_conv_desc* d) {
  dn::IgemmParams p;
  const dn::ConvFamily* f = dn::plan_route(d, &p);
  return f == nullptr ? -1 : (f->weight_layout ? f->weight_layout(p) : 0);
}

int32_t dn_conv_bn_partial_rows(const dn_conv_desc* d) {
  dn::IgemmParams p;
  if (dn::build_plan(d, false, &p) != DN_OK) return -1;
  return (p.M + 127) / 128;
}

int32_t dn_conv_fwd_fuses_reciprocal(const dn_conv_desc* d) {
  dn::IgemmParams p;
  const dn::ConvFamily* f = dn::plan_route(d, &p);
  return (f != nullptr && f->fuses_reciprocal && f->fuses_reciprocal(p)) ? 1 : 0;
}

int32_t dn_conv_dgrad_fuses_bn_sums(const dn_conv_desc* d) {
  dn::IgemmParams p;
  const dn::ConvFamily* f = dn::plan_route(d, &p);
  return f == nullptr ? -1 : ((f->takes_bn_sums && f->takes_bn_sums(d)) ? 1 : 0);
}

int32_t dn_conv_fwd_folds_bn_finalize(const dn_conv_desc* d) {
  dn::IgemmParams p;
  const dn::ConvFamily* f = dn::plan_route(d, &p);
  return f == nullptr ? -1 : ((f->folds_bn_finalize && f->folds_bn_finalize(p)) ? 1 : 0);
}

int32_t dn_conv_dgrad_folds_bn_sums(const dn_conv_desc* d) {
  dn::IgemmParams p;
  const dn::ConvFamily* f = dn::plan_route(d, &p);
  return (f != nullptr && f->takes_bn_sums && f->takes_bn_sums(d) && f->folds_bn_sums(p)) ? 1 : 0;
}

int64_t dn_conv_splitk_workspace_bytes(const dn_conv_desc* d) {
  dn::IgemmParams p;
  const dn::ConvFamily* f = dn::plan_route(d, &p);
  return f != nullptr ? (int64_t)f->splitk_workspace_bytes(p) : -1;
}

int dn_debug_conv_plan(const dn_conv_desc* d, int for_wgrad, int32_t* out, int cap) {
  dn::IgemmParams p;
  int rc = dn::build_plan(d, for_wgrad != 0, &p);
  if (rc != DN_OK) return rc;
  int n = 0;
  auto put = [&](long long v) {
    if (n < cap) out[n] = (int32_t)v;
    ++n;
  };
// ... 20 lines not shown
```

### supervised_dispnet_amd/csrc/dn_pointwise.hip

```cpp
#include "dn_device.h"
#include "dn_fold.h"

namespace dn {

constexpr int kThreads = 256;
constexpr int kMaxReduceBlocks = 4096;

static inline int ew_blocks(long long n_items) {
  long long b = (n_items + kThreads - 1) / kThreads;
  if (b > 4096) b = 4096;
  if (b < 1) b = 1;
  return (int)b;
}

static inline int reduce_blocks(long long rows, int C) {
  int V = (C % 4 == 0) ? 4 : 1;
  int groups = C / V;
  int tpr = 1;
  while (tpr < groups && tpr < kThreads) tpr <<= 1;
  int rpi = kThreads / tpr;
  const int rpt = 2;
  long long b = (rows + (long long)rpi * rpt - 1) / ((long long)rpi * rpt);
  const int cap = 1024 < kMaxReduceBlocks ? 1024 : kMaxReduceBlocks;
  if (b > cap) b = cap;
// ... 213 lines not shown
    pix /= PW;
    const int py = (int)(pix % PH), n = (int)(pix / PH);
    const uchar4 code = *reinterpret_cast<const uchar4*>(idx + i * 4);
    const f32x4 gv = *reinterpret_cast<const f32x4*>(dpooled + i * 4);
    float* base = dx + (((long long)n * H + 2 * py) * W + 2 * px) * C + g * 4;
#pragma unroll
    for (int q = 0; q < 4; ++q) {
      float* dst = base + ((long long)(q >> 1) * W + (q & 1)) * C;
      f32x4 o = accumulate ? *reinterpret_cast<const f32x4*>(dst) : f32x4{0.f, 0.f, 0.f, 0.f};
      if ((code.x & 3) == q) o[0] += gv[0];
      if ((code.y & 3) == q) o[1] += gv[1];
      if ((code.z & 3) == q) o[2] += gv[2];
      if ((code.w & 3) == q) o[3] += gv[3];
      *reinterpret_cast<f32x4*>(dst) = o;
    }
  }
}

struct PoolBwdOp {
  static constexpr int NACC = 2;
  const float* dpooled;
  const uint8_t* idx;
  const float* y;
  const float* mean;
  const float* invstd;
  float* dz;
  int PH, PW, H, W, C;
  template <int V>
  __device__ __forceinline__ void apply(long long row, int c0, float (&acc)[V][2]) const {
    const int px = (int)(row % PW);
    long long t = row / PW;
    const int py = (int)(t % PH), n = (int)(t / PH);
    const Vec<V> dp = ldv<V>(dpooled + row * C + c0);
    const Vec<V> mu = ldv<V>(mean + c0), is = ldv<V>(invstd + c0);
    const long long base = (((long long)n * H + 2 * py) * W + 2 * px) * C + c0;
    Vec<V> out[4];
#pragma unroll
    for (int q = 0; q < 4; ++q)
#pragma unroll
      for (int e = 0; e < V; ++e) out[q].v[e] = 0.f;
    unsigned codes = 0;
    if constexpr (V == 4) codes = *reinterpret_cast<const unsigned*>(idx + row * C + c0);
    Vec<V> yq[4];
#pragma unroll
    for (int q = 0; q < 4; ++q) yq[q] = ldv<V>(y + base + ((long long)(q >> 1) * W + (q & 1)) * C);
#pragma unroll
    for (int e = 0; e < V; ++e) {
      const int code = V == 4 ? (int)((codes >> (8 * e)) & 0xffu) : (int)idx[row * C + c0 + e];
      if (code & 4) {
        const int q = code & 3;
        const float g = dp.v[e];
        const float yv = q == 0 ? yq[0].v[e] : (q == 1 ? yq[1].v[e] : (q == 2 ? yq[2].v[e] : yq[3].v[e]));
#pragma unroll
        for (int qq = 0; qq < 4; ++qq)
          if (qq == q) out[qq].v[e] = g;
        acc[e][0] += g;
        acc[e][1] += g * (yv - mu.v[e]) * is.v[e];
      }
    }
    if (dz != nullptr) {
#pragma unroll
      for (int q = 0; q < 4; ++q) stv<V>(dz + base + ((long long)(q >> 1) * W + (q & 1)) * C, out[q]);
    }
  }
};

struct BnReluBwdOp {
  static constexpr int NACC = 2;
  int write;
  float* da_dz;
  const float* y;
  const float* scale;
  const float* shift;
  const float* mean;
  const float* invstd;
  int C;
  template <int V>
  __device__ __forceinline__ void apply(long long row, int c0, float (&acc)[V][2]) const {
    const long long o = row * C + c0;
    Vec<V> g = ldv<V>(da_dz + o);
    const Vec<V> yv = ldv<V>(y + o), sc = ldv<V>(scale + c0), sh = ldv<V>(shift + c0), mu = ldv<V>(mean + c0), is = ldv<V>(invstd + c0);
#pragma unroll
    for (int e = 0; e < V; ++e) {
      const float dz = (yv.v[e] * sc.v[e] + sh.v[e] > 0.f) ? g.v[e] : 0.f;
      g.v[e] = dz;
      acc[e][0] += dz;
      acc[e][1] += dz * (yv.v[e] - mu.v[e]) * is.v[e];
    }
    if (write) stv<V>(da_dz + o, g);
  }
};

struct ActBwdOp {
  static constexpr int NACC = 1;
  const float* src;
  float* g;
  const float* y_post;
  int act;
  float p0, p1;
  int C;
  template <int V>
  __device__ __forceinline__ void apply(long long row, int c0, float (&acc)[V][1]) const {
    const long long o = row * C + c0;
    Vec<V> gv = ldv<V>(src + o);
    if (act == DN_ACT_NONE) {
      if (src != g) stv<V>(g + o, gv);
    } else {
      const Vec<V> yv = ldv<V>(y_post + o);
#pragma unroll
      for (int e = 0; e < V; ++e) {
        const float yp = yv.v[e];
        float d = 1.f;
        if (act == DN_ACT_RELU) d = yp > 0.f ? 1.f : 0.f;
        else if (act == DN_ACT_LEAKY) d = yp > 0.f ? 1.f : p0;
        else if (act == DN_ACT_ELU) d = yp > 0.f ? 1.f : (yp + 1.f);
        else if (act == DN_ACT_SIGMOID_AFFINE) {
          const float sg = (yp - p1) / p0;
          d = p0 * sg * (1.f - sg);
        }
        gv.v[e] *= d;
      }
      stv<V>(g + o, gv);
    }
#pragma unroll
    for (int e = 0; e < V; ++e) acc[e][0] += gv.v[e];
  }
};

__global__ void __launch_bounds__(256) colsum_finalize_kernel(const float* __restrict__ partial, int rows, int C, int stride, int offset,
                                                              float* __restrict__ out) {
  const int lane = threadIdx.x & 63;
  const int c = blockIdx.x * 4 + (threadIdx.x >> 6);
  if (c >= C) return;
  double s = 0.0;
  for (int r = lane; r < rows; r += 64) s += (double)partial[((long long)r * C + c) * stride + offset];
#pragma unroll
  for (int o = 32; o > 0; o >>= 1) s += __shfl_xor(s, o);
  if (lane == 0) out[c] = (float)s;
}

__global__ void __launch_bounds__(256) colsum2_finalize_kernel(const float* __restrict__ partial, int rows, int C, int stride, int offset,
                                                               float* __restrict__ out0, float* __restrict__ out1) {
  const int c = blockIdx.x;
  double s0 = 0.0, s1 = 0.0;
#pragma unroll 4
  for (int r = threadIdx.x; r < rows; r += 256) {
    const float* q = partial + ((long long)r * C + c) * stride + offset;
    s0 += (double)q[0];
    s1 += (double)q[1];
  }
#pragma unroll
  for (int o = 32; o > 0; o >>= 1) {
    s0 += __shfl_xor(s0, o);
    s1 += __shfl_xor(s1, o);
  }
  __shared__ double red[2][4];
  if ((threadIdx.x & 63) == 0) {
    red[0][threadIdx.x >> 6] = s0;
    red[1][threadIdx.x >> 6] = s1;
  }
  __syncthreads();
  if (threadIdx.x == 0) {
    out0[c] = (float)((red[0][0] + red[0][1]) + (red[0][2] + red[0][3]));
    out1[c] = (float)((red[1][0] + red[1][1]) + (red[1][2] + red[1][3]));
  }
}

__device__ __forceinline__ float bn_bwd_value(float z, float yv, float mu, float is, float ga, float dg, float db, float inv_count) {
#pragma clang fp contract(off)
  const float xhat = (yv - mu) * is;
  float t = __builtin_fmaf(-db, inv_count, z);
  t = __builtin_fmaf(-(xhat * dg), inv_count, t);
  return (ga * is) * t;
}

__global__ void __launch_bounds__(kThreads) bn_bwd_apply_kernel(float* __restrict__ dz_dy, const float* __restrict__ y,
                                                                const float* __restrict__ mean, const float* __restrict__ invstd,
                                                                const float* __restrict__ gamma, const float* __restrict__ dgamma,
                                                                const float* __restrict__ dbeta, long long rows, int C, float inv_count) {
  const int G = C / 4;
  const long long total = rows * G;
  for (long long i = blockIdx.x * (long long)kThreads + threadIdx.x; i < total; i += (long long)gridDim.x * kThreads) {
    const int c = (int)(i % G) * 4;
    const long long o = i * 4;
    f32x4 dz = *reinterpret_cast<const f32x4*>(dz_dy + o);
    const f32x4 yv = *reinterpret_cast<const f32x4*>(y + o);
    const f32x4 mu = *reinterpret_cast<const f32x4*>(mean + c), is = *reinterpret_cast<const f32x4*>(invstd + c);
    const f32x4 ga = *reinterpret_cast<const f32x4*>(gamma + c), dg = *reinterpret_cast<const f32x4*>(dgamma + c),
                db = *reinterpret_cast<const f32x4*>(dbeta + c);
#pragma unroll
    for (int e = 0; e < 4; ++e) {
      dz[e] = bn_bwd_value(dz[e], yv[e], mu[e], is[e], ga[e], dg[e], db[e], inv_count);
    }
    *reinterpret_cast<f32x4*>(dz_dy + o) = dz;
  }
}

__global__ void __launch_bounds__(kThreads) bn_bwd_apply_relu_kernel(float* __restrict__ da_dy, const float* __restrict__ y,
                                                                     const float* __restrict__ scale, const float* __restrict__ shift,
                                                                     const float* __restrict__ mean, const float* __restrict__ invstd,
                                                                     const float* __restrict__ gamma, const float* __restrict__ dgamma,
                                                                     const float* __restrict__ dbeta, long long rows, int C, float inv_count) {
  const int G = C / 4;
  const long long total = rows * G;
  for (long long i = blockIdx.x * (long long)kThreads + threadIdx.x; i < total; i += (long long)gridDim.x * kThreads) {
    const int c = (int)(i % G) * 4;
    const long long o = i * 4;
    f32x4 dz = *reinterpret_cast<const f32x4*>(da_dy + o);
    const f32x4 yv = *reinterpret_cast<const f32x4*>(y + o);
    const f32x4 sc = *reinterpret_cast<const f32x4*>(scale + c), sh = *reinterpret_cast<const f32x4*>(shift + c);
    const f32x4 mu = *reinterpret_cast<const f32x4*>(mean + c), is = *reinterpret_cast<const f32x4*>(invstd + c);
    const f32x4 ga = *reinterpret_cast<const f32x4*>(gamma + c), dg = *reinterpret_cast<const f32x4*>(dgamma + c),
                db = *reinterpret_cast<const f32x4*>(dbeta + c);
#pragma unroll
    for (int e = 0; e < 4; ++e) {
      const float z = (yv[e] * sc[e] + sh[e] > 0.f) ? dz[e] : 0.f;
      dz[e] = bn_bwd_value(z, yv[e], mu[e], is[e], ga[e], dg[e], db[e], inv_count);
    }
    *reinterpret_cast<f32x4*>(da_dy + o) = dz;
  }
}

__global__ void __launch_bounds__(kThreads) bn_bwd_apply_relu_hoisted_kernel(float* __restrict__ da_dy, const float* __restrict__ y,
                                                                             const float* __restrict__ scale, const float* __restrict__ shift,
                                                                             const float* __restrict__ mean, const float* __restrict__ invstd,
                                                                             const float* __restrict__ gamma, const float* __restrict__ dgamma,
                                                                             const float* __restrict__ dbeta, long long rows, int C, float inv_count) {
  const int G = C / 4;
  const long long total = rows * G;
  const int c = (int)(threadIdx.x % (unsigned)G) * 4;
  const f32x4 sc = *reinterpret_cast<const f32x4*>(scale + c), sh = *reinterpret_cast<const f32x4*>(shift + c);
  const f32x4 mu = *reinterpret_cast<const f32x4*>(mean + c), is = *reinterpret_cast<const f32x4*>(invstd + c);
  const f32x4 ga = *reinterpret_cast<const f32x4*>(gamma + c), dg = *reinterpret_cast<const f32x4*>(dgamma + c),
              db = *reinterpret_cast<const f32x4*>(dbeta + c);
  const long long step = (long long)gridDim.x * kThreads;
  for (long long i0 = blockIdx.x * (long long)kThreads + threadIdx.x; i0 < total; i0 += 4 * step) {
    f32x4 dz[4], yv[4];
#pragma unroll
    for (int u = 0; u < 4; ++u) {
      const long long i = i0 + u * step;
      if (i < total) {
        dz[u] = __builtin_nontemporal_load(reinterpret_cast<const f32x4*>(da_dy + i * 4));
        yv[u] = __builtin_nontemporal_load(reinterpret_cast<const f32x4*>(y + i * 4));
      }
    }
#pragma unroll
    for (int u = 0; u < 4; ++u) {
      const long long i = i0 + u * step;
      if (i < total) {
#pragma unroll
        for (int e = 0; e < 4; ++e) {
          const float z = (yv[u][e] * sc[e] + sh[e] > 0.f) ? dz[u][e] : 0.f;
          dz[u][e] = bn_bwd_value(z, yv[u][e], mu[e], is[e], ga[e], dg[e], db[e], inv_count);
        }
        *reinterpret_cast<f32x4*>(da_dy + i * 4) = dz[u];
      }
    }
  }
}

__global__ void __launch_bounds__(kThreads) bn_bwd_apply_hoisted_kernel(float* __restrict__ dz_dy, const float* __restrict__ y,
                                                                        const float* __restrict__ mean, const float* __restrict__ invstd,
                                                                        const float* __restrict__ gamma, const float* __restrict__ dgamma,
                                                                        const float* __restrict__ dbeta, long long rows, int C, float inv_count) {
  const int G = C / 4;
  const long long total = rows * G;
  const long long first = blockIdx.x * (long long)kThreads + threadIdx.x;
  const int c = (int)(first % G) * 4;
  const f32x4 mu = *reinterpret_cast<const f32x4*>(mean + c), is = *reinterpret_cast<const f32x4*>(invstd + c);
  const f32x4 ga = *reinterpret_cast<const f32x4*>(gamma + c), dg = *reinterpret_cast<const f32x4*>(dgamma + c),
              db = *reinterpret_cast<const f32x4*>(dbeta + c);
  const long long step = (long long)gridDim.x * kThreads;
  for (long long i0 = first; i0 < total; i0 += 4 * step) {
    f32x4 dz[4], yv[4];
#pragma unroll
    for (int u = 0; u < 4; ++u) {
      const long long i = i0 + u * step;
      if (i < total) {
        dz[u] = __builtin_nontemporal_load(reinterpret_cast<const f32x4*>(dz_dy + i * 4));
        yv[u] = __builtin_nontemporal_load(reinterpret_cast<const f32x4*>(y + i * 4));
      }
    }
#pragma unroll
    for (int u = 0; u < 4; ++u) {
      const long long i = i0 + u * step;
      if (i < total) {
#pragma unroll
        for (int e = 0; e < 4; ++e) dz[u][e] = bn_bwd_value(dz[u][e], yv[u][e], mu[e], is[e], ga[e], dg[e], db[e], inv_count);
        *reinterpret_cast<f32x4*>(dz_dy + i * 4) = dz[u];
      }
    }
  }
}

__global__ void __launch_bounds__(kThreads) bn_bwd_apply_pool_kernel(const float* __restrict__ dpooled, const uint8_t* __restrict__ idx,
                                                                     const float* __restrict__ y, const float* __restrict__ mean,
                                                                     const float* __restrict__ invstd, const float* __restrict__ gamma,
                                                                     const float* __restrict__ dgamma, const float* __restrict__ dbeta, int N,
                                                                     int H, int W, int C, float inv_count, float* __restrict__ dy) {
  const int G = C / 4, PH = H / 2, PW = W / 2;
  const long long total = (long long)N * PH * PW * G;
  for (long long i = blockIdx.x * (long long)kThreads + threadIdx.x; i < total; i += (long long)gridDim.x * kThreads) {
    const int g = (int)(i % G);
    long long pix = i / G;
    const int px = (int)(pix % PW);
    pix /= PW;
    const int py = (int)(pix % PH), n = (int)(pix / PH);
    const int c = g * 4;
    const f32x4 dp = *reinterpret_cast<const f32x4*>(dpooled + i * 4);
    const uchar4 code = *reinterpret_cast<const uchar4*>(idx + i * 4);
    const int cd[4] = {code.x, code.y, code.z, code.w};
    const f32x4 mu = *reinterpret_cast<const f32x4*>(mean + c), is = *reinterpret_cast<const f32x4*>(invstd + c);
    const f32x4 ga = *reinterpret_cast<const f32x4*>(gamma + c), dg = *reinterpret_cast<const f32x4*>(dgamma + c),
                db = *reinterpret_cast<const f32x4*>(dbeta + c);
    const long long base = (((long long)n * H + 2 * py) * W + 2 * px) * C + c;
#pragma unroll
    for (int q = 0; q < 4; ++q) {
      const long long o = base + ((long long)(q >> 1) * W + (q & 1)) * C;
      const f32x4 yv = *reinterpret_cast<const f32x4*>(y + o);
      f32x4 out;
#pragma unroll
      for (int e = 0; e < 4; ++e) {
        const float z = ((cd[e] & 4) && (cd[e] & 3) == q) ? dp[e] : 0.f;
        out[e] = bn_bwd_value(z, yv[e], mu[e], is[e], ga[e], dg[e], db[e], inv_count);
      }
      *reinterpret_cast<f32x4*>(dy + o) = out;
    }
  }
}

__global__ void __launch_bounds__(kThreads) bn_add_relu_fwd_kernel(const float* __restrict__ y, const float* __restrict__ scale,
                                                                   const float* __restrict__ shift, const float* __restrict__ r,
                                                                   const float* __restrict__ r_scale, const float* __restrict__ r_shift,
                                                                   long long rows, int C, float* __restrict__ out) {
  const int G = C / 4;
// ... 387 lines not shown
  const long long total = (long long)N * (H / 2) * (W / 2) * (C / 4);
  DN_LAUNCH(bn_relu_pool_fwd_kernel, dim3(ew_blocks(total)), dim3(kThreads), 0, as_stream(stream), y, scale, shift, N, H, W, C,
                     pooled, idx);
  return check_launch("bn_relu_pool_fwd_kernel");
}

int dn_maxpool2_bwd(const float* dpooled, const uint8_t* idx, int32_t N, int32_t H, int32_t W, int32_t C, float* dx, int32_t accumulate,
                    dn_stream_t stream) {
  DN_REQUIRE(dpooled && idx && dx && N > 0, DN_ERR_BAD_ARG, "dn_maxpool2_bwd: bad argument");
  DN_REQUIRE(C % 4 == 0 && H % 2 == 0 && W % 2 == 0, DN_ERR_UNSUPPORTED, "dn_maxpool2_bwd: need C%%4==0 and even H,W");
  const long long total = (long long)N * (H / 2) * (W / 2) * (C / 4);
  DN_LAUNCH(maxpool2_bwd_kernel, dim3(ew_blocks(total)), dim3(kThreads), 0, as_stream(stream), dpooled, idx, N, H, W, C, dx, accumulate);
  return check_launch("maxpool2_bwd_kernel");
}

int dn_bn_relu_pool_bwd(const float* dpooled, const uint8_t* idx, const float* y, const float* mean, const float* invstd, int32_t N,
                        int32_t H, int32_t W, int32_t C, float* dz, float* partial, dn_stream_t stream) {
  DN_REQUIRE(dpooled && idx && y && mean && invstd && dz && partial, DN_ERR_BAD_ARG, "dn_bn_relu_pool_bwd: null pointer");
  DN_REQUIRE(C % 4 == 0 && H % 2 == 0 && W % 2 == 0, DN_ERR_UNSUPPORTED, "dn_bn_relu_pool_bwd: need C%%4==0 and even H,W");
  PoolBwdOp op{dpooled, idx, y, mean, invstd, dz, H / 2, W / 2, H, W, C};
  return launch_colreduce(op, (long long)N * (H / 2) * (W / 2), C, partial, as_stream(stream), "bn_relu_pool_bwd");
}

int dn_bn_relu_pool_bwd_sums(const float* dpooled, const uint8_t* idx, const float* y, const float* mean, const float* invstd, int32_t N,
                             int32_t H, int32_t W, int32_t C, float* partial, dn_stream_t stream) {
  DN_REQUIRE(dpooled && idx && y && mean && invstd && partial, DN_ERR_BAD_ARG, "dn_bn_relu_pool_bwd_sums: null pointer");
  DN_REQUIRE(C % 4 == 0 && H % 2 == 0 && W % 2 == 0, DN_ERR_UNSUPPORTED, "dn_bn_relu_pool_bwd_sums: need C%%4==0 and even H,W");
  PoolBwdOp op{dpooled, idx, y, mean, invstd, nullptr, H / 2, W / 2, H, W, C};
  return launch_colreduce(op, (long long)N * (H / 2) * (W / 2), C, partial, as_stream(stream), "bn_relu_pool_bwd_sums");
}

int dn_bn_relu_bwd_reduce(float* da_dz, const float* y, const float* scale, const float* shift, const float* mean, const float* invstd,
                          int64_t rows, int32_t C, float* partial, dn_stream_t stream) {
  DN_REQUIRE(da_dz && y && scale && shift && mean && invstd && partial && rows > 0 && C > 0, DN_ERR_BAD_ARG,
             "dn_bn_relu_bwd_reduce: bad argument");
  BnReluBwdOp op{1, da_dz, y, scale, shift, mean, invstd, C};
  return launch_colreduce(op, rows, C, partial, as_stream(stream), "bn_relu_bwd_reduce");
}

int dn_bn_relu_bwd_sums(const float* da, const float* y, const float* scale, const float* shift, const float* mean, const float* invstd,
                        int64_t rows, int32_t C, float* partial, dn_stream_t stream) {
  DN_REQUIRE(da && y && scale && shift && mean && invstd && partial && rows > 0 && C > 0, DN_ERR_BAD_ARG, "dn_bn_relu_bwd_sums: bad argument");
  BnReluBwdOp op{0, const_cast<float*>(da), y, scale, shift, mean, invstd, C};
  return launch_colreduce(op, rows, C, partial, as_stream(stream), "bn_relu_bwd_sums");
}

static void launch_colsum2(const float* partial, int32_t partial_rows, int32_t C, int32_t partial_stride, int32_t partial_offset, float* out0,
                           float* out1, hipStream_t s) {
  if (partial_rows <= kFoldMaxRows && (partial_stride & 1) == 0 && (partial_offset & 1) == 0 && (reinterpret_cast<uintptr_t>(partial) & 7) == 0)
    DN_LAUNCH(colsum2_sliced_kernel, dim3((C + 63) / 64), dim3(256), 0, s, partial, partial_rows, C, partial_stride, partial_offset, out0, out1);
  else
    DN_LAUNCH(colsum2_finalize_kernel, dim3(C), dim3(256), 0, s, partial, partial_rows, C, partial_stride, partial_offset, out0, out1);
}

static int bn_bwd_sums_to_params(const float* partial, int32_t partial_rows, int32_t partial_stride, int32_t partial_offset, int32_t C,
                                 float* dgamma, float* dbeta, hipStream_t s, const char* who) {
  DN_REQUIRE(dgamma && dbeta, DN_ERR_BAD_ARG, "%s: bad argument", who);
  DN_REQUIRE(C % 4 == 0, DN_ERR_UNSUPPORTED, "%s: need C%%4==0", who);
  if (partial == nullptr) return DN_OK;
  DN_REQUIRE(partial_rows > 0, DN_ERR_BAD_ARG, "%s: bad argument", who);
  DN_REQUIRE(partial_stride >= 2 && partial_offset >= 0 && partial_offset + 1 < partial_stride, DN_ERR_BAD_ARG, "%s: partial layout", who);
  launch_colsum2(partial, partial_rows, C, partial_stride, partial_offset, dbeta, dgamma, s);
  return DN_OK;
}

int dn_bn_bwd_apply_relu(float* da_dy, const float* y, const float* scale, const float* shift, const float* mean, const float* invstd,
                         const float* gamma, const float* partial, int32_t partial_rows, int32_t partial_stride, int32_t partial_offset,
                         int64_t rows, int32_t C, float* dgamma, float* dbeta, dn_stream_t stream) {
  DN_REQUIRE(da_dy && y && scale && shift && mean && invstd && gamma && rows > 0, DN_ERR_BAD_ARG, "dn_bn_bwd_apply_relu: bad argument");
  hipStream_t s = as_stream(stream);
  int rc = bn_bwd_sums_to_params(partial, partial_rows, partial_stride, partial_offset, C, dgamma, dbeta, s, "dn_bn_bwd_apply_relu");
  if (rc != DN_OK) return rc;
  const bool hoisted = C % 4 == 0 && kThreads % (C / 4) == 0;
  set_last_kernel(hoisted ? "dn::bn_bwd_apply_relu_hoisted_kernel" : "dn::bn_bwd_apply_relu_kernel");
  if (hoisted)
    DN_LAUNCH(bn_bwd_apply_relu_hoisted_kernel, dim3(ew_blocks((rows * (C / 4) + 3) / 4)), dim3(kThreads), 0, s, da_dy, y, scale, shift, mean,
              invstd, gamma, dgamma, dbeta, (long long)rows, C, (float)(1.0 / (double)rows));
  else
    DN_LAUNCH(bn_bwd_apply_relu_kernel, dim3(ew_blocks(rows * (C / 4))), dim3(kThreads), 0, s, da_dy, y, scale, shift, mean, invstd, gamma,
                     dgamma, dbeta, (long long)rows, C, (float)(1.0 / (double)rows));
  return check_launch("bn_bwd_apply_relu");
}

int dn_bn_bwd_apply_pool(const float* dpooled, const uint8_t* idx, const float* y, const float* mean, const float* invstd, const float* gamma,
                         const float* partial, int32_t partial_rows, int32_t partial_stride, int32_t partial_offset, int32_t N, int32_t H,
                         int32_t W, int32_t C, float* dy, float* dgamma, float* dbeta, dn_stream_t stream) {
  DN_REQUIRE(dpooled && idx && y && mean && invstd && gamma && dy && N > 0, DN_ERR_BAD_ARG, "dn_bn_bwd_apply_pool: bad argument");
  DN_REQUIRE(H % 2 == 0 && W % 2 == 0, DN_ERR_UNSUPPORTED, "dn_bn_bwd_apply_pool: need even H, W");
  hipStream_t s = as_stream(stream);
  int rc = bn_bwd_sums_to_params(partial, partial_rows, partial_stride, partial_offset, C, dgamma, dbeta, s, "dn_bn_bwd_apply_pool");
  if (rc != DN_OK) return rc;
  const long long total = (long long)N * (H / 2) * (W / 2) * (C / 4);
  DN_LAUNCH(bn_bwd_apply_pool_kernel, dim3(ew_blocks(total)), dim3(kThreads), 0, s, dpooled, idx, y, mean, invstd, gamma, dgamma, dbeta, N,
                     H, W, C, (float)(1.0 / ((double)N * H * W)), dy);
  return check_launch("bn_bwd_apply_pool");
}

int dn_bn_bwd_apply(float* dz_dy, const float* y, const float* mean, const float* invstd, const float* gamma, const float* partial,
                    int32_t partial_rows, int32_t partial_stride, int32_t partial_offset, int64_t rows, int32_t C, float* dgamma,
                    float* dbeta, dn_stream_t stream) {
  DN_REQUIRE(dz_dy && y && mean && invstd && gamma && partial && dgamma && dbeta && rows > 0, DN_ERR_BAD_ARG, "dn_bn_bwd_apply: bad argument");
  DN_REQUIRE(C % 4 == 0, DN_ERR_UNSUPPORTED, "dn_bn_bwd_apply: need C%%4==0");
  DN_REQUIRE(partial_stride >= 2 && partial_offset >= 0 && partial_offset + 1 < partial_stride, DN_ERR_BAD_ARG, "dn_bn_bwd_apply: partial layout");
  hipStream_t s = as_stream(stream);
  launch_colsum2(partial, partial_rows, C, partial_stride, partial_offset, dbeta, dgamma, s);
  const int G = C / 4;
  int blocks = ew_blocks((rows * (long long)G + 3) / 4);
  int ga = G, gb = kThreads;
  while (gb != 0) {
    const int t = ga % gb;
    ga = gb;
    gb = t;
  }
  const int per = G / ga;
  if (per <= 64) {
    blocks = (blocks + per - 1) / per * per;
    set_last_kernel("dn::bn_bwd_apply_hoisted_kernel");
    DN_LAUNCH(bn_bwd_apply_hoisted_kernel, dim3(blocks), dim3(kThreads), 0, s, dz_dy, y, mean, invstd, gamma, dgamma, dbeta, (long long)rows, C,
              (float)(1.0 / (double)rows));
  } else {
    set_last_kernel("dn::bn_bwd_apply_kernel");
    DN_LAUNCH(bn_bwd_apply_kernel, dim3(ew_blocks(rows * (C / 4))), dim3(kThreads), 0, s, dz_dy, y, mean, invstd, gamma, dgamma, dbeta,
              (long long)rows, C, (float)(1.0 / (double)rows));
  }
  return check_launch("bn_bwd_apply");
}

int dn_act_bwd_reduce(float* g, const float* y_post, int32_t act, float p0, float p1, int64_t rows, int32_t C, float* partial,
                      dn_stream_t stream) {
  DN_REQUIRE(g && partial && rows > 0 && C > 0 && (act == DN_ACT_NONE || y_post), DN_ERR_BAD_ARG, "dn_act_bwd_reduce: bad argument");
  ActBwdOp op{g, g, y_post, act, p0, p1, C};
  return launch_colreduce(op, rows, C, partial, as_stream(stream), "act_bwd_reduce");
}

int dn_act_bwd_reduce_from(const float* g_in, float* g_out, const float* y_post, int32_t act, float p0, float p1, int64_t rows, int32_t C,
                           float* partial, dn_stream_t stream) {
  DN_REQUIRE(g_in && g_out && partial && rows > 0 && C > 0 && (act == DN_ACT_NONE || y_post), DN_ERR_BAD_ARG, "dn_act_bwd_reduce_from: bad argument");
  ActBwdOp op{g_in, g_out, y_post, act, p0, p1, C};
  return launch_colreduce(op, rows, C, partial, as_stream(stream), "act_bwd_reduce_from");
}

int dn_colsum_finalize(const float* partial, int32_t rows, int32_t C, int32_t stride, int32_t offset, float* out, dn_stream_t stream) {
  DN_REQUIRE(partial && out && rows > 0 && C > 0 && stride > 0 && offset >= 0 && offset < stride, DN_ERR_BAD_ARG, "dn_colsum_finalize: bad argument");
  DN_LAUNCH(colsum_finalize_kernel, dim3((C + 3) / 4), dim3(256), 0, as_stream(stream), partial, rows, C, stride, offset, out);
  return check_launch("colsum_finalize_kernel");
}

int dn_upsample2x_nearest_bwd(const float* dfull, int32_t N, int32_t h, int32_t w, float* dlow, int32_t accumulate, dn_stream_t stream) {
  DN_REQUIRE(dfull && dlow && N > 0 && h > 0 && w > 0, DN_ERR_BAD_ARG, "dn_upsample2x_nearest_bwd: bad argument");
  DN_LAUNCH(upsample2x_nearest_bwd_kernel, dim3(ew_blocks((long long)N * h * w)), dim3(256), 0, as_stream(stream), dfull, N, h, w,
                     dlow, accumulate);
  return check_launch("upsample2x_nearest_bwd_kernel");
}

int dn_upsample2x_bilinear_fwd(const float* low, int32_t N, int32_t h, int32_t w, int32_t OH, int32_t OW, float* out, dn_stream_t stream) {
  DN_REQUIRE(low && out && N > 0 && OH <= 2 * h && OW <= 2 * w && OH > 0 && OW > 0, DN_ERR_BAD_ARG, "dn_upsample2x_bilinear_fwd: bad argument");
  DN_LAUNCH(upsample2x_bilinear_fwd_kernel, dim3(ew_blocks((long long)N * OH * OW)), dim3(256), 0, as_stream(stream), low, N, h, w,
                     OH, OW, out);
  return check_launch("upsample2x_bilinear_fwd_kernel");
}

int dn_upsample2x_bilinear_bwd(const float* dout, int32_t N, int32_t h, int32_t w, int32_t OH, int32_t OW, float* dlow, int32_t accumulate,
                               dn_stream_t stream) {
  DN_REQUIRE(dout && dlow && N > 0 && OH <= 2 * h && OW <= 2 * w && OH > 0 && OW > 0, DN_ERR_BAD_ARG, "dn_upsample2x_bilinear_bwd: bad argument");
  DN_LAUNCH(upsample2x_bilinear_bwd_kernel, dim3(ew_blocks((long long)N * h * w)), dim3(256), 0, as_stream(stream), dout, N, h, w,
                     OH, OW, dlow, accumulate);
// ... 143 lines not shown
```

### supervised_dispnet_amd/csrc/dn_wino_common.h

```cpp
#pragma once
#include "dn_device.h"
#include "dn_fold.h"

namespace dn {

constexpr int WBT = 64;
constexpr int WBN = 64;
constexpr int WKC = 16;
constexpr int WZLD = 72;

template <int MTW>
struct WinoCfg {
  static constexpr int BT = 32 * MTW;
  static constexpr int HALFB = BT * 16 + 32;
  static constexpr int POSB = 2 * HALFB;
  static constexpr int SUBB = 16 * POSB + 64;
  static constexpr int BUFB = 2 * SUBB;
  static constexpr size_t LDS = (size_t)2 * BUFB;
};

constexpr int W16_ROWB = 48;

template <int NK, int TSTEP, int NWAVES, int GROUPS>
__device__ __forceinline__ void wino_bn_bwd_sums(const IgemmParams& p, const f32x4 (&Y)[NK][2][2], int mb, int tg, int c4, int wave, int lane, int tid,
                                                 int n_first, float* red) {
  constexpr int BT = 32 * GROUPS;
  f32x4 s1[GROUPS], s2[GROUPS];
#pragma unroll
  for (int g = 0; g < GROUPS; ++g) s1[g] = s2[g] = f32x4{0.f, 0.f, 0.f, 0.f};
  if (n_first < p.Ntot) {
    const f32x4 sc = *reinterpret_cast<const f32x4*>(p.bnb_scale + n_first), sh = *reinterpret_cast<const f32x4*>(p.bnb_shift + n_first);
    const f32x4 mu = *reinterpret_cast<const f32x4*>(p.bnb_mean + n_first), is = *reinterpret_cast<const f32x4*>(p.bnb_invstd + n_first);
    const long long C = p.Ntot, rowB = (long long)p.OW * C;
#pragma unroll
    for (int k = 0; k < NK; ++k) {
      const int t = mb * BT + tg + TSTEP * k;
      if (t < p.T) {
        unsigned tx, ty;
        const unsigned r = fastdiv_dev((unsigned)t, (unsigned)p.TW, p.mTW, &tx);
        const int n = (int)fastdiv_dev(r, (unsigned)p.TH, p.mTH, &ty);
        const float* y00 = p.bnb_y + (((long long)n * p.OH + 2 * (int)ty) * p.OW + 2 * (int)tx) * C + n_first;
        const f32x4 yv[2][2] = {{*reinterpret_cast<const f32x4*>(y00), *reinterpret_cast<const f32x4*>(y00 + C)},
                                {*reinterpret_cast<const f32x4*>(y00 + rowB), *reinterpret_cast<const f32x4*>(y00 + rowB + C)}};
#pragma unroll
        for (int a = 0; a < 2; ++a)
#pragma unroll
          for (int b = 0; b < 2; ++b)
#pragma unroll
            for (int e = 0; e < 4; ++e) {
              const float yy = yv[a][b][e];
              const float dz = (yy * sc[e] + sh[e] > 0.f) ? Y[k][a][b][e] : 0.f;
              s1[(k * TSTEP) / 32][e] += dz;
              s2[(k * TSTEP) / 32][e] += dz * (yy - mu[e]) * is[e];
            }
      }
    }
  }
#pragma unroll
  for (int g = 0; g < GROUPS; ++g)
#pragma unroll
    for (int e = 0; e < 4; ++e) {
      s1[g][e] += __shfl_xor(s1[g][e], 16);
      s1[g][e] += __shfl_xor(s1[g][e], 32);
      s2[g][e] += __shfl_xor(s2[g][e], 16);
      s2[g][e] += __shfl_xor(s2[g][e], 32);
    }
  __syncthreads();
  if (lane < 16) {
#pragma unroll
    for (int g = 0; g < GROUPS; ++g) {
      *reinterpret_cast<f32x4*>(red + ((g * NWAVES + wave) * 2 + 0) * 64 + 4 * c4) = s1[g];
      *reinterpret_cast<f32x4*>(red + ((g * NWAVES + wave) * 2 + 1) * 64 + 4 * c4) = s2[g];
    }
  }
  __syncthreads();
  if (tid < 64 * GROUPS) {
    const int g = tid >> 6, col = tid & 63;
    float a1 = 0.f, a2 = 0.f;
#pragma unroll
    for (int w = 0; w < NWAVES; ++w) {
      a1 += red[((g * NWAVES + w) * 2 + 0) * 64 + col];
      a2 += red[((g * NWAVES + w) * 2 + 1) * 64 + col];
    }
    const int n = (n_first - 4 * c4) + col;
    if (n < p.Ntot && mb * BT + 32 * g < p.T) {
      float* dst = p.bnb_partial + ((long long)(GROUPS * mb + g) * p.Ntot + n) * 2;
      fold_store(dst, a1);
      fold_store(dst + 1, a2);
    }
  }
}

__device__ __forceinline__ void wino_fold_tail(const IgemmParams& p, int nb, int mblocks, float* lds, int tid) {
  if (!(p.fold_bn | p.fold_bnb)) return;
  __shared__ int fold_flag;
  if (!fold_last_arrival(p.fold_cnt + nb, mblocks, &fold_flag)) return;
  const int rows = (p.T + 31) / 32, c0 = nb * WBN;
  const int nlive = p.Ntot - c0 < WBN ? p.Ntot - c0 : WBN;
  double* red = reinterpret_cast<double*>(lds);
  if (p.fold_bn) bn_finalize_sliced<true>(p.bn_partial, rows, p.Ntot, c0, nlive, (double)p.M, p.bnf, red, tid);
  if (p.fold_bnb) colsum2_sliced<true>(p.bnb_partial, rows, p.Ntot, 2, 0, c0, nlive, p.bnb_dbeta, p.bnb_dgamma, red, tid);
}

bool wino8_wanted(const IgemmParams& p);
int launch_wino_conv8(const IgemmParams& p, hipStream_t stream);

}
```

### supervised_dispnet_amd/engine.py

```python
import ctypes as C
import math
import os
import threading
import weakref

import torch

from . import _lib
from ._lib import (ACT_LEAKY, ACT_NONE, ACT_RELU, ACT_SIGMOID_AFFINE, CONV_DGRAD, CONV_FWD, CONVT_DGRAD, CONVT_FWD,
                   ConvDesc)

BN_EPS = 1e-5
BN_MOMENTUM = 0.1

PARAM_EPOCH = 0


PROFILE = None

SPLITK = True
PACK_ON_SIDE_STREAM = True
PACK_LATE_MIN_ELEMS = 400000
BN_SUMS_FUSION = True
FOLD_FINALIZE = True
BN_MATERIALIZE_DZ = False

COMPUTE_MODES = {"f32": _lib.COMPUTE_F32, "bf16": _lib.COMPUTE_BF16, "f32x3": _lib.COMPUTE_F32X3}
if os.environ.get("DN_COMPUTE", "f32x3").lower() not in COMPUTE_MODES:
    raise ValueError("DN_COMPUTE=%r: expected one of %s" % (os.environ["DN_COMPUTE"], sorted(COMPUTE_MODES)))
COMPUTE = COMPUTE_MODES[os.environ.get("DN_COMPUTE", "f32x3").lower()]


def set_compute(mode):
    global COMPUTE
    if mode not in COMPUTE_MODES:
        raise ValueError("compute mode is one of %s, got %r" % (sorted(COMPUTE_MODES), mode))
    COMPUTE = COMPUTE_MODES[mode]
    bump_param_epoch()


def compute_mode():
    return [k for k, v in COMPUTE_MODES.items() if v == COMPUTE][0]


CAPTURING = False


_WGRAD_STREAM_MODE = os.environ.get("DN_WGRAD_STREAM", "auto")
WGRAD_STREAM = _WGRAD_STREAM_MODE != "0"
WGRAD_STREAMS = 2
WGRAD_STREAMS_MAX_PIXELS = 16 * 128 * 416
SIDE_STREAMS_ACTIVE = 1


def choose_side_streams(input_pixels):
    global SIDE_STREAMS_ACTIVE
    SIDE_STREAMS_ACTIVE = WGRAD_STREAMS if input_pixels <= WGRAD_STREAMS_MAX_PIXELS else 1
_SIDE = {}


def wgrad_stream_enabled():
    if _WGRAD_STREAM_MODE == "0" or PROFILE is not None:
        return False
    return True


def side_stream():
    dev = torch.cuda.current_device()
    st = _SIDE.get(dev)
    if st is None:
        sides = [torch.cuda.Stream(device=dev) for _ in range(max(1, WGRAD_STREAMS))]
        st = _SIDE[dev] = {"side": sides[0], "sides": sides, "handles": {x.cuda_stream for x in sides}, "main": None, "rr": 0}
    return st


TAPE = None
DEVICE_SCOPE_FENCES = True
BORROW_SEED_GRADS = True


def stream_wait(waiter, waitee, device_scope=False):
    waiter.wait_stream(waitee)
    if TAPE is not None and not TAPE.get("paused"):
        _lib.call("dn_tape_fence_device" if (device_scope and DEVICE_SCOPE_FENCES) else "dn_tape_fence", TAPE["handle"], waiter.cuda_stream,
                  waitee.cuda_stream)


def tape_host_call(fn):
    if TAPE is None:
        return fn()
    _lib.load().dn_tape_mark(TAPE["handle"])
    TAPE["host_calls"].append((fn, torch.cuda.current_stream()))
    _lib.call("dn_tape_pause", TAPE["handle"], 1)
    TAPE["paused"] = True
    try:
        return fn()
    finally:
        TAPE["paused"] = False
        _lib.call("dn_tape_pause", TAPE["handle"], 0)


class outside_tape_pool(object):

    def __enter__(self):
        self.rec = TAPE
        if self.rec is not None and self.rec.get("pool") is not None:
            torch._C._cuda_endAllocateToPool(*self.rec["pool"])
# ... 465 lines not shown
        h = _stream()
        if h == side.cuda_stream:
            return
        stream_wait(main if h == main.cuda_stream else torch.cuda.current_stream(), side, device_scope=True)
        self.pending = None


_PACK_TABLES = {}


def pack_table(device):
    t = _PACK_TABLES.get(device)
    if t is None:
        t = _PACK_TABLES[device] = PackTable(device)
    return t


def prepack_all(device):
    t = _PACK_TABLES.get(device)
    if t is not None:
        t.run(PARAM_EPOCH)


FUSE_RECIP = True


def conv_forward(layer, pieces, act=ACT_NONE, p0=0.0, p1=0.0, bn_stats=False, out_hw=None, out_view=None, recip=None, bn_fold=None):
    a0 = pieces[0].act
    N = a0.N
    IH = a0.H * (2 if pieces[0].up else 1)
    IW = a0.W * (2 if pieces[0].up else 1)
    OH, OW = out_hw or layer.out_size(IH, IW)
    kind = CONVT_FWD if layer.transposed else CONV_FWD
    d = layer._desc(kind, N, IH, IW, OH, OW)
    d.n_in = len(pieces)
    for i, p in enumerate(pieces):
        _fill_operand(d.in_[i], p)
    d.n_out = 1
    if out_view is None:
        y = torch.empty((N, OH, OW, layer.Cout), dtype=torch.float32, device=a0.t.device)
        _fill_result(d.out[0], y, layer.Cout, OH, OW, False)
    else:
        y, off, (vsn, vsh, vsw), vacc = out_view
        r = d.out[0]
        r.data = y.data_ptr() + 4 * off
        r.C = layer.Cout
        r.accumulate = 1 if vacc else 0
        r.stride_n, r.stride_h, r.stride_w = vsn, vsh, vsw
    d.w_packed = layer.packed(kind, d).data_ptr()
    b = layer.m.bias
    d.bias = _ptr(b.detach()) if b is not None else None
    d.act, d.act_p0, d.act_p1 = act, p0, p1
    _splitk_workspace(d, a0.t.device)
    partial, rows = None, 0
    if recip is not None and out_view is None and layer.Cout == 1 and _lib.load().dn_conv_fwd_fuses_reciprocal(C.byref(d)) == 1:
        recip.append(torch.empty((N, OH, OW, 1), dtype=torch.float32, device=a0.t.device))
        d.recip_out = recip[0].data_ptr()
    if bn_stats:
        rows = _lib.load().dn_conv_bn_partial_rows(C.byref(d))
        partial = torch.empty((rows, layer.Cout, 2), dtype=torch.float32, device=y.device)
        d.bn_partial = partial.data_ptr()
        if bn_fold is not None and FOLD_FINALIZE and d.splitk_ws:
            bn = bn_fold[0]
            d.bnf_gamma, d.bnf_beta = bn.weight.data_ptr(), bn.bias.data_ptr()
            d.bnf_running_mean, d.bnf_running_var = _ptr(bn.running_mean), _ptr(bn.running_var)
            d.bnf_num_batches_tracked = bn_fold[5]
            d.bnf_momentum = bn.momentum if bn.momentum is not None else BN_MOMENTUM
            d.bnf_eps = bn.eps
            d.bnf_mean, d.bnf_invstd, d.bnf_scale, d.bnf_shift = (t.data_ptr() for t in bn_fold[1:5])
            if _lib.load().dn_conv_fwd_folds_bn_finalize(C.byref(d)) == 1:
                bn_fold[0] = True
            else:
                d.bnf_scale = None
    if bn_fold is not None and bn_fold[0] is not True:
        bn_fold[0] = False
    with _Timed("igemm_conv_kernel<128,%d>" % _pick_bn(layer.Cout), 2 * layer.macs(N, IH, IW, OH, OW),
                "%s %dx%d k%d s%d cin%d cout%d in %dx%dx%d" % ("convT_fwd" if layer.transposed else "conv_fwd", layer.R, layer.S,
                                                               layer.R, layer.stride, layer.Cin, layer.Cout, N, IH, IW),
                4 * (sum(p.act.rows * p.act.C for p in pieces) + N * OH * OW * layer.Cout)):
        _lib.call("dn_convT2d_fwd" if layer.transposed else "dn_conv2d_fwd", C.byref(d), _stream())
    return y, partial, rows


def conv_wgrad(layer, pieces, dy, out_hw, out=None, sink=None, first=None):
    a0 = pieces[0].act
    IH = a0.H * (2 if pieces[0].up else 1)
    IW = a0.W * (2 if pieces[0].up else 1)
    OH, OW = out_hw
    kind = CONVT_FWD if layer.transposed else CONV_FWD
    d = layer._desc(kind, a0.N, IH, IW, OH, OW)
    d.n_in = len(pieces)
    for i, p in enumerate(pieces):
        _fill_operand(d.in_[i], p)
    d.n_out = 1
    d.out[0].C = layer.Cout
    lib = _lib.load()
    nbytes = lib.dn_conv_wgrad_workspace_bytes(C.byref(d))
    if nbytes == 0:
        raise _lib.DispnetHipError("dn_conv_wgrad_workspace_bytes: " + _lib.last_error())

    def launch():
        ws = torch.empty(nbytes // 4, dtype=torch.float32, device=dy.device)
        dw = out if out is not None else torch.empty_like(layer.m.weight, memory_format=torch.contiguous_format)
        with _Timed("igemm_wgrad_kernel<%d>" % _pick_bn(layer.Cin if layer.transposed else layer.Cout),
                    2 * layer.macs(a0.N, IH, IW, OH, OW),
                    "%s k%d s%d cin%d cout%d in %dx%dx%d" % ("convT_wgrad" if layer.transposed else "conv_wgrad", layer.R, layer.stride,
                                                             layer.Cin, layer.Cout, a0.N, IH, IW),
                    4 * (sum(p.act.rows * p.act.C for p in pieces) + dy.numel())):
            _lib.call("dn_conv2d_wgrad", C.byref(d), dy.data_ptr(), dw.data_ptr(), ws.data_ptr(), nbytes, _stream())
        if sink is not None:
            sink.put(layer.m.weight, dw)
        return dw

    if not (dy.is_cuda and wgrad_stream_enabled()):
        if first is not None:
            first[0]()
        return launch()
    st = side_stream()
    main = torch.cuda.current_stream()
    side = st["sides"][st["rr"] % min(len(st["sides"]), max(1, SIDE_STREAMS_ACTIVE))]
    st["rr"] += 1
    st["main"] = main
    stream_wait(side, main, device_scope=True)
    with stream_scope(side):
        if first is not None:
            fresh = first[0]()
            cross_stream_use(first[1], side)
            if fresh is not None:
                cross_stream_use(fresh, main)
        dw = launch()
    cross_stream_use(dy, side)
    for p in pieces:
        cross_stream_use(p.act.t, side)
        if p.act.scale is not None:
            cross_stream_use(p.act.scale, side)
            cross_stream_use(p.act.shift, side)
    if out is None:
        cross_stream_use(dw, main)
    return dw


def conv_dgrad(layer, dy, N, OH, OW, pieces, in_hw):
    targets = [p for p in pieces]
    if not any(p.act.needs_grad for p in targets):
        return
    IH, IW = in_hw
    kind = CONVT_DGRAD if layer.transposed else CONV_DGRAD
    rp = layer.pad if layer.reflect else 0
    GH, GW = IH + 2 * rp, IW + 2 * rp
    d = layer._desc(kind, N, OH, OW, GH, GW)
    if layer.reflect:
        d.pad = 0
    d.n_in = 1
    op = d.in_[0]
    op.data = dy.data_ptr()
    op.C = layer.Cout
    op.up_shift = 0
    op.stride_c, op.stride_w, op.stride_h, op.stride_n = 1, layer.Cout, OW * layer.Cout, OH * OW * layer.Cout
    d.n_out = len(targets)
    post = []
    for i, p in enumerate(targets):
        a = p.act
        if p.up or layer.reflect:
            tmp = torch.empty((N, GH, GW, a.C), dtype=torch.float32, device=dy.device)
            _fill_result(d.out[i], tmp, a.C, GH, GW, False)
            if a.needs_grad:
                post.append((p, tmp))
        elif not a.needs_grad:
            tmp = torch.empty((N, IH, IW, a.C), dtype=torch.float32, device=dy.device)
            _fill_result(d.out[i], tmp, a.C, IH, IW, False)
        else:
            first = a.grad is None
            if first:
                a.grad = a.new_like()
            else:
                a.sums_ready = False
                a.sums_final = None
            _fill_result(d.out[i], a.grad, a.C, IH, IW, not first)
    d.w_packed = layer.packed(kind, d).data_ptr()
    d.bias = None
    d.act = ACT_NONE
    _splitk_workspace(d, dy.device)
    fuse = None
    if BN_SUMS_FUSION and len(targets) == 1 and not layer.transposed and not layer.reflect:
        a = targets[0].act
        if (not targets[0].up and a.needs_grad and a.scale is not None and a.mean is not None and not a.no_relu and not a.grad_is_dz
                and d.out[0].accumulate == 0 and a.strides == (a.H * a.W * a.C, a.W * a.C, a.C, 1)):
            d.bnb_y, d.bnb_scale, d.bnb_shift = a.t.data_ptr(), a.scale.data_ptr(), a.shift.data_ptr()
            d.bnb_mean, d.bnb_invstd = a.mean.data_ptr(), a.invstd.data_ptr()
            rows = _lib.load().dn_conv_bn_partial_rows(C.byref(d))
            scratch = torch.empty((max(rows, 1), a.C, 2), dtype=torch.float32, device=dy.device)
            d.bnb_partial = scratch.data_ptr()
            if _lib.load().dn_conv_dgrad_fuses_bn_sums(C.byref(d)) == 1:
                fuse = (a, scratch, rows, None)
                if FOLD_FINALIZE and a.bn_owner is not None and d.splitk_ws:
                    obn, osink = a.bn_owner
                    dg, db = osink.dest(obn.weight), osink.dest(obn.bias)
                    if dg is None:
                        dg = torch.empty(a.C, dtype=torch.float32, device=dy.device)
                    if db is None:
                        db = torch.empty(a.C, dtype=torch.float32, device=dy.device)
                    d.bnb_dgamma, d.bnb_dbeta = dg.data_ptr(), db.data_ptr()
                    if _lib.load().dn_conv_dgrad_folds_bn_sums(C.byref(d)) == 1:
                        fuse = (a, scratch, rows, (dg, db))
                    else:
                        d.bnb_dgamma = d.bnb_dbeta = None
            else:
                d.bnb_y = d.bnb_partial = None
    with _Timed("igemm_conv_kernel<128,%d>" % _pick_bn(layer.Cin), 2 * layer.macs(N, IH, IW, OH, OW),
                "%s k%d s%d cin%d cout%d in %dx%dx%d" % ("convT_dgrad" if layer.transposed else "conv_dgrad", layer.R, layer.stride,
                                                         layer.Cin, layer.Cout, N, IH, IW),
                4 * (dy.numel() + sum(p.act.rows * p.act.C for p in targets))):
        _lib.call("dn_convT2d_dgrad" if layer.transposed else "dn_conv2d_dgrad", C.byref(d), _stream())
    if fuse is not None:
# ... 12 lines not shown
                first = a.grad is None
                if first:
                    a.grad = a.new_like()
                _lib.call("dn_reflect_fold", tmp.data_ptr(), N, IH, IW, a.C, rp, a.grad.data_ptr(), 0 if first else 1, _stream())
                continue
        first = a.grad is None
        if first:
            a.grad = a.new_like()
        if a.C == 1:
            _lib.call("dn_upsample2x_nearest_bwd", cur.data_ptr(), N, a.H, a.W, a.grad.data_ptr(), 0 if first else 1, _stream())
        else:
            _lib.call("dn_upsample2x_nearest_bwd_nhwc", cur.data_ptr(), N, a.H, a.W, a.C, a.grad.data_ptr(), 0 if first else 1, _stream())


def colsum(partial, rows, Cn, stride=1, offset=0, out=None):
    if out is None:
        out = torch.empty(Cn, dtype=torch.float32, device=partial.device)
    _lib.call("dn_colsum_finalize", partial.data_ptr(), rows, Cn, stride, offset, out.data_ptr(), _stream())
    return out


def act_bwd(g, y_post, act, p0, p1, rows, Cn, out=None, defer=False, src=None):
    nblk = _lib.load().dn_reduce_blocks(rows, Cn)
    partial = torch.empty((nblk, Cn), dtype=torch.float32, device=g.device)
    kname = "dn::colreduce_kernel<dn::ActBwdOp, %d>" % (4 if Cn % 4 == 0 else 1)
    if src is not None:
        hbm_call(kname, rows * Cn * 12, "dn_act_bwd_reduce_from", src.data_ptr(), g.data_ptr(), _ptr(y_post), act, p0, p1, rows, Cn,
                 partial.data_ptr(), _stream())
    else:
        hbm_call(kname, rows * Cn * 12, "dn_act_bwd_reduce", g.data_ptr(), _ptr(y_post), act, p0, p1, rows, Cn, partial.data_ptr(), _stream())
    if defer:
        return (lambda: colsum(partial, nblk, Cn, out=out)), partial
    return colsum(partial, nblk, Cn, out=out)


class GradSink:

    reducer = None

    def __init__(self):
        self.grads = {}

    @staticmethod
    def dest(param):
        return getattr(param, "_dn_grad_view", None)

    def put(self, param, g):
        dst = getattr(param, "_dn_grad_view", None)
        if dst is not None:
            if g.data_ptr() != dst.data_ptr():
                dst.copy_(g.view_as(dst))
            param._dn_zero_grad_slot = False
            self.grads[id(param)] = None
            if GradSink.reducer is not None:
                GradSink.reducer.grad_ready(param)
        else:
            self.grads[id(param)] = g

    def put_zero(self, param):
        dst = getattr(param, "_dn_grad_view", None)
        if dst is not None:
            if not getattr(param, "_dn_zero_grad_slot", False):
                _lib.call("dn_fill", dst.data_ptr(), 0.0, dst.numel(), _stream())
                param._dn_zero_grad_slot = True
            self.grads[id(param)] = None
            if GradSink.reducer is not None:
                GradSink.reducer.grad_ready(param)
        else:
            self.grads[id(param)] = torch.zeros_like(param)

    def put_none(self, param):
        if getattr(param, "_dn_grad_view", None) is not None:
            self.put_zero(param)

    def settle(self, params):
        for p in params:
            if id(p) not in self.grads and getattr(p, "_dn_grad_view", None) is not None and p.requires_grad:
                self.put_zero(p)

    def get(self, param):
        return self.grads.get(id(param))


def bn_backward(y, bn, sink, training):
    g, y_t, Cn, dev = y.grad, y.t, y.C, y.t.device
    if not training:
        raise NotImplementedError("backward through eval-mode BatchNorm (frozen statistics) is not implemented")
    relu_pending = not y.grad_is_dz
    final = None
    if relu_pending and y.sums_ready and not BN_MATERIALIZE_DZ:
        y.sums_ready = False
        final, y.sums_final = y.sums_final, None
    elif relu_pending:
        y.sums_ready = False
        if y.no_relu:
            raise RuntimeError("a ReLU-less BatchNorm output must be consumed by block_bn_add_relu / block_bn_plain")
        nblk = _lib.load().dn_reduce_blocks(y.rows, Cn)
        y.partial = torch.empty((nblk, Cn, 2), dtype=torch.float32, device=dev)
        y.partial_rows = nblk
        if BN_MATERIALIZE_DZ:
            hbm_call("dn::colreduce_kernel<dn::BnReluBwdOp, 4>", y.rows * Cn * 12, "dn_bn_relu_bwd_reduce", g.data_ptr(),
                     y_t.data_ptr(), y.scale.data_ptr(), y.shift.data_ptr(), y.mean.data_ptr(), y.invstd.data_ptr(), y.rows, Cn,
                     y.partial.data_ptr(), _stream())
        else:
            hbm_call("dn::colreduce_kernel<dn::BnReluBwdOp, 4>", y.rows * Cn * 8, "dn_bn_relu_bwd_sums", g.data_ptr(),
                     y_t.data_ptr(), y.scale.data_ptr(), y.shift.data_ptr(), y.mean.data_ptr(), y.invstd.data_ptr(), y.rows, Cn,
                     y.partial.data_ptr(), _stream())
    if final is not None:
        dgamma, dbeta = final
    else:
        dgamma = sink.dest(bn.weight)
        dbeta = sink.dest(bn.bias)
        if dgamma is None:
            dgamma = torch.empty(Cn, dtype=torch.float32, device=dev)
        if dbeta is None:
            dbeta = torch.empty(Cn, dtype=torch.float32, device=dev)
    if y.pool_src is not None:
        dpooled, pidx = y.pool_src
        hbm_call("dn::bn_bwd_apply_pool_kernel", y.rows * Cn * 8 + y.rows * Cn * 5 // 4, "dn_bn_bwd_apply_pool", dpooled.data_ptr(),
                 pidx.data_ptr(), y_t.data_ptr(), y.mean.data_ptr(), y.invstd.data_ptr(), bn.weight.data_ptr(), y.partial.data_ptr(),
                 y.partial_rows, y.partial_stride, y.partial_offset, y.N, y.H, y.W, Cn, g.data_ptr(), dgamma.data_ptr(),
                 dbeta.data_ptr(), _stream())
        y.pool_src = None
    elif relu_pending and not BN_MATERIALIZE_DZ:
        hbm_call(None, y.rows * Cn * 12, "dn_bn_bwd_apply_relu", g.data_ptr(), y_t.data_ptr(),
                 y.scale.data_ptr(), y.shift.data_ptr(), y.mean.data_ptr(), y.invstd.data_ptr(), bn.weight.data_ptr(),
                 None if final is not None else y.partial.data_ptr(), y.partial_rows, y.partial_stride, y.partial_offset, y.rows, Cn,
                 dgamma.data_ptr(), dbeta.data_ptr(), _stream())
    else:
        hbm_call(None, y.rows * Cn * 12, "dn_bn_bwd_apply", g.data_ptr(), y_t.data_ptr(), y.mean.data_ptr(),
                 y.invstd.data_ptr(), bn.weight.data_ptr(), y.partial.data_ptr(), y.partial_rows, y.partial_stride,
                 y.partial_offset, y.rows, Cn, dgamma.data_ptr(), dbeta.data_ptr(), _stream())
    sink.put(bn.weight, dgamma)
    sink.put(bn.bias, dbeta)
    return g


def _bn_pending(y, bn, partial, prow, training, conv_bias=None):
    Cn, dev = y.C, y.t.device
    y.scale = torch.empty(Cn, dtype=torch.float32, device=dev)
    y.shift = torch.empty(Cn, dtype=torch.float32, device=dev)
    if training:
        y.mean = torch.empty(Cn, dtype=torch.float32, device=dev)
        y.invstd = torch.empty(Cn, dtype=torch.float32, device=dev)
        _lib.call("dn_bn_finalize", partial.data_ptr(), prow, Cn, y.rows, _ptr(conv_bias.detach()) if conv_bias is not None else None,
                  bn.weight.data_ptr(), bn.bias.data_ptr(), bn.running_mean.data_ptr(), bn.running_var.data_ptr(),
                  bn.momentum if bn.momentum is not None else BN_MOMENTUM, bn.eps, y.mean.data_ptr(), y.invstd.data_ptr(),
                  y.scale.data_ptr(), y.shift.data_ptr(), _nbt_ptr(bn), _stream())
    else:
        _lib.call("dn_bn_eval_affine", Cn, bn.weight.data_ptr(), bn.bias.data_ptr(), bn.running_mean.data_ptr(),
                  bn.running_var.data_ptr(), bn.eps, y.scale.data_ptr(), y.shift.data_ptr(), _stream())


def block_conv_bn(tape, sink, x_piece, layer, bn, training, relu=True):
    xa = x_piece.act
    dev = xa.t.device
    Cn = layer.Cout
    scale = torch.empty(Cn, dtype=torch.float32, device=dev)
    shift = torch.empty(Cn, dtype=torch.float32, device=dev)
    mean = invstd = fold = nbt = None
    if training:
        mean = torch.empty(Cn, dtype=torch.float32, device=dev)
        invstd = torch.empty(Cn, dtype=torch.float32, device=dev)
        nbt = _nbt_ptr(bn)
        fold = [bn, mean, invstd, scale, shift, nbt]
    y_t, partial, prow = conv_forward(layer, [x_piece], ACT_NONE, bn_stats=training, bn_fold=fold)
    OH, OW = y_t.shape[1], y_t.shape[2]
    y = Act(y_t, xa.N, OH, OW, Cn)
    y.no_relu = not relu
    y.scale, y.shift, y.mean, y.invstd = scale, shift, mean, invstd
    y.bn_owner = (bn, sink)
    if training:
        if fold[0] is not True:
            _lib.call("dn_bn_finalize", partial.data_ptr(), prow, Cn, y.rows, _ptr(layer.m.bias.detach()) if layer.m.bias is not None else None,
                      bn.weight.data_ptr(), bn.bias.data_ptr(), bn.running_mean.data_ptr(), bn.running_var.data_ptr(),
                      bn.momentum if bn.momentum is not None else BN_MOMENTUM, bn.eps, y.mean.data_ptr(), y.invstd.data_ptr(),
                      y.scale.data_ptr(), y.shift.data_ptr(), nbt, _stream())
    else:
        _lib.call("dn_bn_eval_affine", Cn, bn.weight.data_ptr(), bn.bias.data_ptr(), bn.running_mean.data_ptr(),
                  bn.running_var.data_ptr(), bn.eps, y.scale.data_ptr(), y.shift.data_ptr(), _stream())

    def backward():
        if y.grad is None:
            return
        g = bn_backward(y, bn, sink, training)
        if layer.m.bias is not None:
            sink.put_zero(layer.m.bias)
        conv_wgrad(layer, [x_piece], g, (OH, OW), out=sink.dest(layer.m.weight), sink=sink)
        conv_dgrad(layer, g, xa.N, OH, OW, [x_piece], (xa.H, xa.W))
        y.grad = None

    tape.push(backward)
    return y


def block_pool(tape, y):
    dev = y.t.device
    p_t = torch.empty((y.N, y.H // 2, y.W // 2, y.C), dtype=torch.float32, device=dev)
    idx = torch.empty((y.N, y.H // 2, y.W // 2, y.C), dtype=torch.uint8, device=dev)
    hbm_call("dn::bn_relu_pool_fwd_kernel", y.rows * y.C * 4 * 1.25 + y.rows * y.C // 4, "dn_bn_relu_pool_fwd", y.t.data_ptr(),
             y.scale.data_ptr(), y.shift.data_ptr(), y.N, y.H, y.W, y.C, p_t.data_ptr(), idx.data_ptr(), _stream())
    p = Act(p_t, y.N, y.H // 2, y.W // 2, y.C)

    def backward():
        if p.grad is None:
            return
        nblk = _lib.load().dn_reduce_blocks(p.rows, y.C)
        y.partial = torch.empty((nblk, y.C, 2), dtype=torch.float32, device=dev)
        y.partial_rows = nblk
        y.grad = y.new_like()
        y.grad_is_dz = True
        if BN_MATERIALIZE_DZ:
            hbm_call("dn::colreduce_kernel<dn::PoolBwdOp, 4>", y.rows * y.C * 4 * 2.25 + y.rows * y.C // 4, "dn_bn_relu_pool_bwd",
                     p.grad.data_ptr(), idx.data_ptr(), y.t.data_ptr(), y.mean.data_ptr(), y.invstd.data_ptr(), y.N, y.H, y.W, y.C,
                     y.grad.data_ptr(), y.partial.data_ptr(), _stream())
        else:
            hbm_call("dn::colreduce_kernel<dn::PoolBwdOp, 4>", y.rows * y.C * 4 * 1.25 + y.rows * y.C // 4, "dn_bn_relu_pool_bwd_sums",
                     p.grad.data_ptr(), idx.data_ptr(), y.t.data_ptr(), y.mean.data_ptr(), y.invstd.data_ptr(), y.N, y.H, y.W, y.C,
                     y.partial.data_ptr(), _stream())
            y.pool_src = (p.grad, idx)
        p.grad = None

    tape.push(backward)
    return p


def block_conv_act(tape, sink, pieces, layer, act, p0=0.0, p1=0.0, out_hw=None, stat_bn=None):
    a0 = pieces[0].act
    in_hw = (a0.H * (2 if pieces[0].up else 1), a0.W * (2 if pieces[0].up else 1))
    want_recip = [] if (FUSE_RECIP and act == ACT_SIGMOID_AFFINE and layer.Cout == 1 and stat_bn is None and p1 > 0) else None
    y_t, partial, prow = conv_forward(layer, pieces, act, p0, p1, out_hw=out_hw, bn_stats=stat_bn is not None, recip=want_recip)
    OH, OW = y_t.shape[1], y_t.shape[2]
    y = Act(y_t, a0.N, OH, OW, layer.Cout)
    if want_recip:
        y.recip_t = want_recip[0]
    if stat_bn is not None:
        Cn, dev = layer.Cout, y_t.device
        scratch = torch.empty((4, Cn), dtype=torch.float32, device=dev)
        _lib.call("dn_bn_finalize", partial.data_ptr(), prow, Cn, y.rows, _ptr(layer.m.bias.detach()) if layer.m.bias is not None else None,
                  stat_bn.weight.data_ptr(), stat_bn.bias.data_ptr(), stat_bn.running_mean.data_ptr(), stat_bn.running_var.data_ptr(),
                  stat_bn.momentum if stat_bn.momentum is not None else BN_MOMENTUM, stat_bn.eps, scratch[0].data_ptr(),
                  scratch[1].data_ptr(), scratch[2].data_ptr(), scratch[3].data_ptr(), _nbt_ptr(stat_bn), _stream())

    def backward():
        if y.grad is None:
            sink.put_none(layer.m.weight)
            if layer.m.bias is not None:
                sink.put_none(layer.m.bias)
            return
        g, g_src = y.grad, None
        if y.grad_borrowed:
            g_src, g, y.grad_borrowed = g, torch.empty_like(y.grad), False
        finish_db, db_partial = act_bwd(g, y_t, act, p0, p1, y.rows, layer.Cout,
                                        out=sink.dest(layer.m.bias) if layer.m.bias is not None else None, defer=True, src=g_src)

        def bias_grad():
            db = finish_db()
            if layer.m.bias is not None:
                sink.put(layer.m.bias, db)
            return db if (layer.m.bias is None or sink.dest(layer.m.bias) is None) else None

        conv_wgrad(layer, pieces, g, (OH, OW), out=sink.dest(layer.m.weight), sink=sink, first=(bias_grad, db_partial))
        conv_dgrad(layer, g, a0.N, OH, OW, pieces, in_hw)
        y.grad = None

    tape.push(backward, out=y)
    return y


def _not_on_tape(what):
    if TAPE is not None and not TAPE.get("paused"):
# ... 410 lines not shown
```

Before: 1992.

## Fuse BatchNorm-ReLU backward apply into stem conv weight-gradient kernel

For the stem convolution, whose input needs no gradient, the BN+ReLU backward apply is now done inside the lds3 stem wgrad kernel. The kernel loads y alongside the incoming gradient and computes dx per element before the bf16 three-way split. This replaces the separate elementwise bn_bwd_apply_relu pass, which read and wrote the full-resolution activation gradient, with a small dgamma/dbeta finalize launch. In exchange the wgrad kernel loads an extra tensor and uses more registers, which may lower its occupancy.

```diff
diff --git a/include/dispnet_hip.h b/include/dispnet_hip.h
--- a/include/dispnet_hip.h
+++ b/include/dispnet_hip.h
@@ -120,6 +120,10 @@
 size_t dn_conv_wgrad_workspace_bytes(const dn_conv_desc* fwd);
 int dn_conv2d_wgrad(const dn_conv_desc* fwd, const float* dy, float* dw, void* workspace, size_t workspace_bytes,
                     dn_stream_t stream);
+int32_t dn_conv_wgrad_applies_bn_relu_bwd(const dn_conv_desc* fwd);
+int dn_conv2d_wgrad_bn_relu(const dn_conv_desc* fwd, const float* da, const float* y, const float* scale, const float* shift,
+                            const float* mean, const float* invstd, const float* gamma, const float* dgamma, const float* dbeta,
+                            int64_t count, float* dw, void* workspace, size_t workspace_bytes, dn_stream_t stream);
 
 int dn_bn_finalize(const float* partial, int32_t rows, int32_t C, int64_t count, const float* conv_bias,
                    const float* gamma, const float* beta, float* running_mean, float* running_var, float momentum,
@@ -146,6 +150,8 @@
 int dn_bn_bwd_apply_relu(float* da_dy, const float* y, const float* scale, const float* shift, const float* mean, const float* invstd,
                          const float* gamma, const float* partial, int32_t partial_rows, int32_t partial_stride, int32_t partial_offset,
                          int64_t rows, int32_t C, float* dgamma, float* dbeta, dn_stream_t stream);
+int dn_bn_bwd_sums_finalize(const float* partial, int32_t partial_rows, int32_t partial_stride, int32_t partial_offset, int32_t C,
+                            float* dgamma, float* dbeta, dn_stream_t stream);
 int dn_bn_bwd_apply_pool(const float* dpooled, const uint8_t* idx, const float* y, const float* mean, const float* invstd, const float* gamma,
                          const float* partial, int32_t partial_rows, int32_t partial_stride, int32_t partial_offset, int32_t N, int32_t H,
                          int32_t W, int32_t C, float* dy, float* dgamma, float* dbeta, dn_stream_t stream);
diff --git a/supervised_dispnet_amd/_lib.py b/supervised_dispnet_amd/_lib.py
--- a/supervised_dispnet_amd/_lib.py
+++ b/supervised_dispnet_amd/_lib.py
@@ -5,7 +5,7 @@
 _PKG = pathlib.Path(__file__).resolve().parent
 LIB_PATH = pathlib.Path(os.environ.get("DISPNET_HIP_LIB", _PKG / "libdispnet_hip.so"))
 
-EXPECTED_ABI = 21
+EXPECTED_ABI = 22
 
 DN_MAX_OPERANDS = 3
 ACT_NONE, ACT_RELU, ACT_LEAKY, ACT_ELU, ACT_SIGMOID_AFFINE = 0, 1, 2, 3, 4
@@ -70,12 +70,15 @@
     "dn_convT2d_dgrad": (C.c_int, [_P(ConvDesc), _vp]),
     "dn_conv_wgrad_workspace_bytes": (_sz, [_P(ConvDesc)]),
     "dn_conv2d_wgrad": (C.c_int, [_P(ConvDesc), _vp, _vp, _vp, _sz, _vp]),
+    "dn_conv_wgrad_applies_bn_relu_bwd": (_i32, [_P(ConvDesc)]),
+    "dn_conv2d_wgrad_bn_relu": (C.c_int, [_P(ConvDesc), _vp, _vp, _vp, _vp, _vp, _vp, _vp, _vp, _vp, _i64, _vp, _vp, _sz, _vp]),
     "dn_bn_finalize": (C.c_int, [_vp, _i32, _i32, _i64, _vp, _vp, _vp, _vp, _vp, _f, _f, _vp, _vp, _vp, _vp, _vp, _vp]),
     "dn_bn_eval_affine": (C.c_int, [_i32, _vp, _vp, _vp, _vp, _f, _vp, _vp, _vp]),
     "dn_bn_relu_pool_fwd": (C.c_int, [_vp, _vp, _vp, _i32, _i32, _i32, _i32, _vp, _vp, _vp]),
     "dn_bn_relu_bwd_sums": (C.c_int, [_vp, _vp, _vp, _vp, _vp, _vp, _i64, _i32, _vp, _vp]),
     "dn_bn_relu_pool_bwd_sums": (C.c_int, [_vp, _vp, _vp, _vp, _vp, _i32, _i32, _i32, _i32, _vp, _vp]),
     "dn_bn_bwd_apply_relu": (C.c_int, [_vp, _vp, _vp, _vp, _vp, _vp, _vp, _vp, _i32, _i32, _i32, _i64, _i32, _vp, _vp, _vp]),
+    "dn_bn_bwd_sums_finalize": (C.c_int, [_vp, _i32, _i32, _i32, _i32, _vp, _vp, _vp]),
     "dn_bn_bwd_apply_pool": (C.c_int, [_vp, _vp, _vp, _vp, _vp, _vp, _vp, _i32, _i32, _i32, _i32, _i32, _i32, _i32, _vp, _vp, _vp, _vp]),
     "dn_maxpool2_bwd": (C.c_int, [_vp, _vp, _i32, _i32, _i32, _i32, _vp, _i32, _vp]),
     "dn_bn_relu_pool_bwd": (C.c_int, [_vp, _vp, _vp, _vp, _vp, _i32, _i32, _i32, _i32, _vp, _vp, _vp]),
diff --git a/supervised_dispnet_amd/csrc/dn_conv.hip b/supervised_dispnet_amd/csrc/dn_conv.hip
--- a/supervised_dispnet_amd/csrc/dn_conv.hip
+++ b/supervised_dispnet_amd/csrc/dn_conv.hip
@@ -2271,6 +2271,15 @@
      [](const dn_conv_desc*, IgemmParams& p, float* dw, hipStream_t s) { return launch_thin_wgrad(p, dw, s); }},
 };
 
+static const WgradFamily* wgrad_route(const dn_conv_desc* fwd, const IgemmParams& p, const float* dy, size_t workspace_bytes) {
+  for (const WgradFamily& f : kWgradFamilies) {
+    if (!f.eligible(fwd, p) || (f.switched_off && f.switched_off()) || workspace_bytes < f.workspace_bytes(fwd, p)) continue;
+    if (f.dy_aligned16 && (reinterpret_cast<uintptr_t>(dy) & 15) != 0) continue;
+    return &f;
+  }
+  return nullptr;
+}
+
 extern "C" {
 
 int64_t dn_pack_entry_bytes(void) { return (int64_t)sizeof(PackEntry); }
@@ -2366,13 +2375,11 @@
   if (rc != DN_OK) return rc;
   DN_REQUIRE(dy != nullptr && dw != nullptr && workspace != nullptr, DN_ERR_BAD_ARG, "null pointer");
   const hipStream_t s = as_stream(stream);
-  for (const WgradFamily& f : kWgradFamilies) {
-    if (!f.eligible(fwd, p) || (f.switched_off && f.switched_off()) || workspace_bytes < f.workspace_bytes(fwd, p)) continue;
-    if (f.dy_aligned16 && (reinterpret_cast<uintptr_t>(dy) & 15) != 0) continue;
+  if (const WgradFamily* f = wgrad_route(fwd, p, dy, workspace_bytes)) {
     for (int i = 0; i < p.n_in; ++i) DN_REQUIRE(p.in[i].p != nullptr, DN_ERR_BAD_ARG, "operand %d has no data", i);
     p.g = dy;
     p.ws = reinterpret_cast<float*>(workspace);
-    return f.launch(fwd, p, dw, s);
+    return f->launch(fwd, p, dw, s);
   }
   {
     dn_conv_desc d1, d2;
@@ -2403,4 +2410,39 @@
   return generic_wgrad(fwd, p, dy, dw, workspace, workspace_bytes, s);
 }
 
-}
+static bool wgrad_routes_to_bn_bwd_kernel(const dn_conv_desc* fwd, const IgemmParams& p, const float* dy, size_t workspace_bytes) {
+  const WgradFamily* f = wgrad_route(fwd, p, dy, workspace_bytes);
+  return f != nullptr && f->launch == launch_lds3_wgrad && lds3_wgrad_applies_bn_bwd(fwd, p);
+}
+
+int32_t dn_conv_wgrad_applies_bn_relu_bwd(const dn_conv_desc* fwd) {
+  IgemmParams p;
+  int rc = build_plan(fwd, true, &p);
+  if (rc != DN_OK) return rc;
+  return wgrad_routes_to_bn_bwd_kernel(fwd, p, nullptr, dn_conv_wgrad_workspace_bytes(fwd)) ? 1 : 0;
+}
+
+int dn_conv2d_wgrad_bn_relu(const dn_conv_desc* fwd, const float* da, const float* y, const float* scale, const float* shift,
+                            const float* mean, const float* invstd, const float* gamma, const float* dgamma, const float* dbeta,
+                            int64_t count, float* dw, void* workspace, size_t workspace_bytes, dn_stream_t stream) {
+  IgemmParams p;
+  int rc = build_plan(fwd, true, &p);
+  if (rc != DN_OK) return rc;
+  DN_REQUIRE(da && y && scale && shift && mean && invstd && gamma && dgamma && dbeta && dw && workspace, DN_ERR_BAD_ARG,
+             "dn_conv2d_wgrad_bn_relu: null pointer");
+  DN_REQUIRE(count == (int64_t)p.M, DN_ERR_BAD_ARG, "dn_conv2d_wgrad_bn_relu: count %lld is not N*OH*OW = %d", (long long)count, p.M);
+  DN_REQUIRE(wgrad_routes_to_bn_bwd_kernel(fwd, p, da, workspace_bytes), DN_ERR_UNSUPPORTED,
+             "dn_conv2d_wgrad_bn_relu: this call does not run on the kernel that applies the BatchNorm backward "
+             "(dn_conv_wgrad_applies_bn_relu_bwd, 16-byte aligned da, the whole workspace)");
+  const uintptr_t al = reinterpret_cast<uintptr_t>(y) | reinterpret_cast<uintptr_t>(scale) | reinterpret_cast<uintptr_t>(shift) |
+                       reinterpret_cast<uintptr_t>(mean) | reinterpret_cast<uintptr_t>(invstd) | reinterpret_cast<uintptr_t>(gamma) |
+                       reinterpret_cast<uintptr_t>(dgamma) | reinterpret_cast<uintptr_t>(dbeta);
+  DN_REQUIRE((al & 15) == 0, DN_ERR_UNSUPPORTED, "dn_conv2d_wgrad_bn_relu: y and the per-channel vectors must be 16-byte aligned");
+  for (int i = 0; i < p.n_in; ++i) DN_REQUIRE(p.in[i].p != nullptr, DN_ERR_BAD_ARG, "operand %d has no data", i);
+  p.g = da;
+  p.ws = reinterpret_cast<float*>(workspace);
+  const BnBwdApplyArgs bnb{y, scale, shift, mean, invstd, gamma, dgamma, dbeta, (long long)count};
+  return launch_lds3_wgrad_bn(fwd, p, &bnb, dw, as_stream(stream));
+}
+
+}
diff --git a/supervised_dispnet_amd/csrc/dn_device.h b/supervised_dispnet_amd/csrc/dn_device.h
--- a/supervised_dispnet_amd/csrc/dn_device.h
+++ b/supervised_dispnet_amd/csrc/dn_device.h
@@ -57,6 +57,16 @@
     default: break;
   }
   return r;
+}
+
+__device__ __forceinline__ bool bn_relu_live(float yv, float scale, float shift) { return yv * scale + shift > 0.f; }
+
+__device__ __forceinline__ float bn_bwd_value(float z, float yv, float mu, float is, float ga, float dg, float db, float inv_count) {
+#pragma clang fp contract(off)
+  const float xhat = (yv - mu) * is;
+  float t = __builtin_fmaf(-db, inv_count, z);
+  t = __builtin_fmaf(-(xhat * dg), inv_count, t);
+  return (ga * is) * t;
 }
 
 __device__ __forceinline__ void split3(const float (&v)[8], bf16x8& h, bf16x8& m, bf16x8& l) {
diff --git a/supervised_dispnet_amd/csrc/dn_internal.h b/supervised_dispnet_amd/csrc/dn_internal.h
--- a/supervised_dispnet_amd/csrc/dn_internal.h
+++ b/supervised_dispnet_amd/csrc/dn_internal.h
@@ -247,6 +247,12 @@
 bool lds3_wgrad_eligible(const dn_conv_desc* fwd, const IgemmParams& p);
 size_t lds3_wgrad_workspace_bytes(const IgemmParams& p);
 int launch_lds3_wgrad(const dn_conv_desc* fwd, IgemmParams& p, float* dw, hipStream_t stream);
+struct BnBwdApplyArgs {
+  const float *y, *scale, *shift, *mean, *invstd, *gamma, *dgamma, *dbeta;
+  long long count;
+};
+bool lds3_wgrad_applies_bn_bwd(const dn_conv_desc* fwd, const IgemmParams& p);
+int launch_lds3_wgrad_bn(const dn_conv_desc* fwd, IgemmParams& p, const BnBwdApplyArgs* bnb, float* dw, hipStream_t stream);
 bool lds3k_wgrad_eligible(const dn_conv_desc* fwd, const IgemmParams& p);
 size_t lds3k_wgrad_workspace_bytes(const IgemmParams& p);
 int launch_lds3k_wgrad(const dn_conv_desc* fwd, IgemmParams& p, float* dw, hipStream_t stream);
diff --git a/supervised_dispnet_amd/csrc/dn_lds3_wgrad.hip b/supervised_dispnet_amd/csrc/dn_lds3_wgrad.hip
--- a/supervised_dispnet_amd/csrc/dn_lds3_wgrad.hip
+++ b/supervised_dispnet_amd/csrc/dn_lds3_wgrad.hip
@@ -222,7 +222,13 @@
 constexpr int WS_IPLANE = 10 * WS_ICOLS;
 constexpr int WGS_LDS = 3 * WS_GPIECE + 3 * WS_IPLANE * 4;
 
-__global__ void __launch_bounds__(256, 2) lds3_wgrad_stem_kernel(const IgemmParams p, const WgGeo geo) {
+struct StemBnBwd {
+  const float *y, *scale, *shift, *mean, *invstd, *gamma, *dgamma, *dbeta;
+  float inv_count;
+};
+
+template <bool BNB>
+__global__ void __launch_bounds__(256, 2) lds3_wgrad_stem_kernel(const IgemmParams p, const WgGeo geo, const StemBnBwd bn) {
   extern __shared__ __align__(16) char lds[];
   char* Gp = lds;
   float* Ip = reinterpret_cast<float*>(lds + 3 * WS_GPIECE);
@@ -250,17 +256,34 @@
 
   f32x4 vg[8];
   float vi[4];
+  f32x4 vy[BNB ? 8 : 1];
+  unsigned vok = 0;
+  f32x4 sc, sh, mu, is, ga, dg, db;
+  __amdgpu_buffer_rsrc_t ry = rg;
+  if constexpr (BNB) {
+    ry = __builtin_amdgcn_make_buffer_rsrc(const_cast<float*>(bn.y), 0, 0x80000000u, 0x00020000);
+    const int c = 4 * (tid >> 4);
+    sc = *reinterpret_cast<const f32x4*>(bn.scale + c), sh = *reinterpret_cast<const f32x4*>(bn.shift + c);
+    mu = *reinterpret_cast<const f32x4*>(bn.mean + c), is = *reinterpret_cast<const f32x4*>(bn.invstd + c);
+    ga = *reinterpret_cast<const f32x4*>(bn.gamma + c), dg = *reinterpret_cast<const f32x4*>(bn.dgamma + c);
+    db = *reinterpret_cast<const f32x4*>(bn.dbeta + c);
+  }
   auto issue_g = [&](int t, int h) __attribute__((always_inline)) {
     const int txb = t % geo.tilesX, q1 = t / geo.tilesX;
     const int tyb = q1 % geo.tilesY, n = q1 / geo.tilesY;
     const int pxg = tid & 15, cq = tid >> 4, row = pxg >> 2, cgp = pxg & 3;
     const int gy = tyb * WG_TH + 4 * h + row;
+    if constexpr (BNB) vok = 0;
 #pragma unroll
     for (int i = 0; i < 8; ++i) {
       const int gx = txb * WG_TW + 8 * cgp + i;
       const bool ok = gy < p.GH && gx < p.GW;
       const int off = (((n * p.GH + gy) * p.GW + gx) * p.Ntot + 4 * cq) * 4;
       vg[i] = __builtin_bit_cast(f32x4, __builtin_amdgcn_raw_buffer_load_b128(rg, ok ? off : -1, 0, 0));
+      if constexpr (BNB) {
+        vy[i] = __builtin_bit_cast(f32x4, __builtin_amdgcn_raw_buffer_load_b128(ry, ok ? off : -1, 0, 0));
+        vok |= (ok ? 1u : 0u) << i;
+      }
     }
   };
   auto issue_img = [&](int t) __attribute__((always_inline)) {
@@ -281,7 +304,15 @@
     const int pxg = tid & 15, cq = tid >> 4;
 #pragma unroll
     for (int e = 0; e < 4; ++e) {
-      const float v[8] = {vg[0][e], vg[1][e], vg[2][e], vg[3][e], vg[4][e], vg[5][e], vg[6][e], vg[7][e]};
+      float v[8] = {vg[0][e], vg[1][e], vg[2][e], vg[3][e], vg[4][e], vg[5][e], vg[6][e], vg[7][e]};
+      if constexpr (BNB) {
+#pragma unroll
+        for (int i = 0; i < 8; ++i) {
+          const float z = bn_relu_live(vy[i][e], sc[e], sh[e]) ? v[i] : 0.f;
+          const float dx = bn_bwd_value(z, vy[i][e], mu[e], is[e], ga[e], dg[e], db[e], bn.inv_count);
+          v[i] = (vok >> i & 1u) ? dx : 0.f;
+        }
+      }
       bf16x8 h, m, l;
       split3(v, h, m, l);
       char* dst = Gp + (4 * cq + e) * WS_GSTR + pxg * 16;
@@ -383,6 +414,8 @@
   return 0;
 }
 
+bool lds3_wgrad_applies_bn_bwd(const dn_conv_desc* d, const IgemmParams& p) { return lds3_wgrad_form(d, p) == 3; }
+
 static int lds3_wgrad_blocks(const IgemmParams& p) {
   const int ntiles = p.N * ((p.GH + WG_TH - 1) / WG_TH) * ((p.GW + WG_TW - 1) / WG_TW);
   int blocks = ntiles < 512 ? ntiles : 512;
@@ -396,7 +429,15 @@
 }
 
 int launch_lds3_wgrad(const dn_conv_desc* d, IgemmParams& p, float* dw, hipStream_t stream) {
+  return launch_lds3_wgrad_bn(d, p, nullptr, dw, stream);
+}
+
+int launch_lds3_wgrad_bn(const dn_conv_desc* d, IgemmParams& p, const BnBwdApplyArgs* bnb, float* dw, hipStream_t stream) {
   const int form = lds3_wgrad_form(d, p);
+  if (bnb != nullptr && form != 3) {
+    set_error("launch_lds3_wgrad: only the stem form applies a pending BatchNorm backward");
+    return DN_ERR_UNSUPPORTED;
+  }
   WgGeo geo;
   geo.tilesX = (p.GW + WG_TW - 1) / WG_TW;
   geo.tilesY = (p.GH + WG_TH - 1) / WG_TH;
@@ -412,9 +453,18 @@
     if (e == hipSuccess) DN_LAUNCH((lds3_wgrad16_kernel<true, true>), dim3(blocks), dim3(256), (size_t)WG16_LDS, stream, p, geo);
     set_last_kernel("dn::lds3_wgrad16_kernel<true>");
   } else if (form == 3) {
-    e = hipFuncSetAttribute(reinterpret_cast<const void*>(lds3_wgrad_stem_kernel), hipFuncAttributeMaxDynamicSharedMemorySize, WGS_LDS);
-    if (e == hipSuccess) DN_LAUNCH(lds3_wgrad_stem_kernel, dim3(blocks), dim3(256), (size_t)WGS_LDS, stream, p, geo);
-    set_last_kernel("dn::lds3_wgrad_stem_kernel");
+    StemBnBwd sb{};
+    if (bnb != nullptr) {
+      sb = StemBnBwd{bnb->y, bnb->scale, bnb->shift, bnb->mean, bnb->invstd, bnb->gamma, bnb->dgamma, bnb->dbeta,
+                     (float)(1.0 / (double)bnb->count)};
+      e = hipFuncSetAttribute(reinterpret_cast<const void*>(lds3_wgrad_stem_kernel<true>), hipFuncAttributeMaxDynamicSharedMemorySize, WGS_LDS);
+      if (e == hipSuccess) DN_LAUNCH(lds3_wgrad_stem_kernel<true>, dim3(blocks), dim3(256), (size_t)WGS_LDS, stream, p, geo, sb);
+      set_last_kernel("dn::lds3_wgrad_stem_kernel<true>");
+    } else {
+      e = hipFuncSetAttribute(reinterpret_cast<const void*>(lds3_wgrad_stem_kernel<false>), hipFuncAttributeMaxDynamicSharedMemorySize, WGS_LDS);
+      if (e == hipSuccess) DN_LAUNCH(lds3_wgrad_stem_kernel<false>, dim3(blocks), dim3(256), (size_t)WGS_LDS, stream, p, geo, sb);
+      set_last_kernel("dn::lds3_wgrad_stem_kernel<false>");
+    }
   } else if (form == 2) {
     e = hipFuncSetAttribute(reinterpret_cast<const void*>(lds3_wgrad16_kernel<true>), hipFuncAttributeMaxDynamicSharedMemorySize, WG16_LDS);
     if (e == hipSuccess) DN_LAUNCH(lds3_wgrad16_kernel<true>, dim3(blocks), dim3(256), (size_t)WG16_LDS, stream, p, geo);
diff --git a/supervised_dispnet_amd/csrc/dn_plan.hip b/supervised_dispnet_amd/csrc/dn_plan.hip
--- a/supervised_dispnet_amd/csrc/dn_plan.hip
+++ b/supervised_dispnet_amd/csrc/dn_plan.hip
@@ -378,7 +378,7 @@
 
 extern "C" {
 
-int dn_version(void) { return 21; }
+int dn_version(void) { return 22; }
 
 void dn_reload_knobs(void) {
   std::lock_guard<std::mutex> lock(dn::g_knobs_mu);
diff --git a/supervised_dispnet_amd/csrc/dn_pointwise.hip b/supervised_dispnet_amd/csrc/dn_pointwise.hip
--- a/supervised_dispnet_amd/csrc/dn_pointwise.hip
+++ b/supervised_dispnet_amd/csrc/dn_pointwise.hip
@@ -319,7 +319,7 @@
     const Vec<V> yv = ldv<V>(y + o), sc = ldv<V>(scale + c0), sh = ldv<V>(shift + c0), mu = ldv<V>(mean + c0), is = ldv<V>(invstd + c0);
 #pragma unroll
     for (int e = 0; e < V; ++e) {
-      const float dz = (yv.v[e] * sc.v[e] + sh.v[e] > 0.f) ? g.v[e] : 0.f;
+      const float dz = bn_relu_live(yv.v[e], sc.v[e], sh.v[e]) ? g.v[e] : 0.f;
       g.v[e] = dz;
       acc[e][0] += dz;
       acc[e][1] += dz * (yv.v[e] - mu.v[e]) * is.v[e];
@@ -403,14 +403,6 @@
   }
 }
 
-__device__ __forceinline__ float bn_bwd_value(float z, float yv, float mu, float is, float ga, float dg, float db, float inv_count) {
-#pragma clang fp contract(off)
-  const float xhat = (yv - mu) * is;
-  float t = __builtin_fmaf(-db, inv_count, z);
-  t = __builtin_fmaf(-(xhat * dg), inv_count, t);
-  return (ga * is) * t;
-}
-
 __global__ void __launch_bounds__(kThreads) bn_bwd_apply_kernel(float* __restrict__ dz_dy, const float* __restrict__ y,
                                                                 const float* __restrict__ mean, const float* __restrict__ invstd,
                                                                 const float* __restrict__ gamma, const float* __restrict__ dgamma,
@@ -451,7 +443,7 @@
                 db = *reinterpret_cast<const f32x4*>(dbeta + c);
 #pragma unroll
     for (int e = 0; e < 4; ++e) {
-      const float z = (yv[e] * sc[e] + sh[e] > 0.f) ? dz[e] : 0.f;
+      const float z = bn_relu_live(yv[e], sc[e], sh[e]) ? dz[e] : 0.f;
       dz[e] = bn_bwd_value(z, yv[e], mu[e], is[e], ga[e], dg[e], db[e], inv_count);
     }
     *reinterpret_cast<f32x4*>(da_dy + o) = dz;
@@ -487,7 +479,7 @@
       if (i < total) {
 #pragma unroll
         for (int e = 0; e < 4; ++e) {
-          const float z = (yv[u][e] * sc[e] + sh[e] > 0.f) ? dz[u][e] : 0.f;
+          const float z = bn_relu_live(yv[u][e], sc[e], sh[e]) ? dz[u][e] : 0.f;
           dz[u][e] = bn_bwd_value(z, yv[u][e], mu[e], is[e], ga[e], dg[e], db[e], inv_count);
         }
         *reinterpret_cast<f32x4*>(da_dy + i * 4) = dz[u];
@@ -1041,6 +1033,14 @@
   return check_launch("bn_bwd_apply_relu");
 }
 
+int dn_bn_bwd_sums_finalize(const float* partial, int32_t partial_rows, int32_t partial_stride, int32_t partial_offset, int32_t C,
+                            float* dgamma, float* dbeta, dn_stream_t stream) {
+  DN_REQUIRE(partial, DN_ERR_BAD_ARG, "dn_bn_bwd_sums_finalize: bad argument");
+  int rc = bn_bwd_sums_to_params(partial, partial_rows, partial_stride, partial_offset, C, dgamma, dbeta, as_stream(stream), "dn_bn_bwd_sums_finalize");
+  if (rc != DN_OK) return rc;
+  return check_launch("bn_bwd_sums_finalize");
+}
+
 int dn_bn_bwd_apply_pool(const float* dpooled, const uint8_t* idx, const float* y, const float* mean, const float* invstd, const float* gamma,
                          const float* partial, int32_t partial_rows, int32_t partial_stride, int32_t partial_offset, int32_t N, int32_t H,
                          int32_t W, int32_t C, float* dy, float* dgamma, float* dbeta, dn_stream_t stream) {
diff --git a/supervised_dispnet_amd/csrc/dn_wino_common.h b/supervised_dispnet_amd/csrc/dn_wino_common.h
--- a/supervised_dispnet_amd/csrc/dn_wino_common.h
+++ b/supervised_dispnet_amd/csrc/dn_wino_common.h
@@ -49,7 +49,7 @@
 #pragma unroll
             for (int e = 0; e < 4; ++e) {
               const float yy = yv[a][b][e];
-              const float dz = (yy * sc[e] + sh[e] > 0.f) ? Y[k][a][b][e] : 0.f;
+              const float dz = bn_relu_live(yy, sc[e], sh[e]) ? Y[k][a][b][e] : 0.f;
               s1[(k * TSTEP) / 32][e] += dz;
               s2[(k * TSTEP) / 32][e] += dz * (yy - mu[e]) * is[e];
             }
diff --git a/supervised_dispnet_amd/engine.py b/supervised_dispnet_amd/engine.py
--- a/supervised_dispnet_amd/engine.py
+++ b/supervised_dispnet_amd/engine.py
@@ -23,6 +23,7 @@
 PACK_LATE_MIN_ELEMS = 400000
 BN_SUMS_FUSION = True
 FOLD_FINALIZE = True
+STEM_WGRAD_APPLIES_BN = True
 BN_MATERIALIZE_DZ = False
 
 COMPUTE_MODES = {"f32": _lib.COMPUTE_F32, "bf16": _lib.COMPUTE_BF16, "f32x3": _lib.COMPUTE_F32X3}
@@ -654,18 +655,34 @@
     return y, partial, rows
 
 
-def conv_wgrad(layer, pieces, dy, out_hw, out=None, sink=None, first=None):
+def _wgrad_desc(layer, pieces, out_hw):
     a0 = pieces[0].act
     IH = a0.H * (2 if pieces[0].up else 1)
     IW = a0.W * (2 if pieces[0].up else 1)
     OH, OW = out_hw
-    kind = CONVT_FWD if layer.transposed else CONV_FWD
-    d = layer._desc(kind, a0.N, IH, IW, OH, OW)
+    d = layer._desc(CONVT_FWD if layer.transposed else CONV_FWD, a0.N, IH, IW, OH, OW)
     d.n_in = len(pieces)
     for i, p in enumerate(pieces):
         _fill_operand(d.in_[i], p)
     d.n_out = 1
     d.out[0].C = layer.Cout
+    return d
+
+
+def wgrad_applies_bn(layer, x_piece, y):
+    if not STEM_WGRAD_APPLIES_BN or BN_MATERIALIZE_DZ or layer.transposed or layer.reflect or x_piece.act.needs_grad:
+        return False
+    if y.grad_is_dz or y.no_relu or y.pool_src is not None or y.strides != (y.H * y.W * y.C, y.W * y.C, y.C, 1):
+        return False
+    return _lib.load().dn_conv_wgrad_applies_bn_relu_bwd(C.byref(_wgrad_desc(layer, [x_piece], (y.H, y.W)))) == 1
+
+
+def conv_wgrad(layer, pieces, dy, out_hw, out=None, sink=None, first=None, bn=None):
+    a0 = pieces[0].act
+    IH = a0.H * (2 if pieces[0].up else 1)
+    IW = a0.W * (2 if pieces[0].up else 1)
+    OH, OW = out_hw
+    d = _wgrad_desc(layer, pieces, out_hw)
     lib = _lib.load()
     nbytes = lib.dn_conv_wgrad_workspace_bytes(C.byref(d))
     if nbytes == 0:
@@ -679,8 +696,17 @@
                     "%s k%d s%d cin%d cout%d in %dx%dx%d" % ("convT_wgrad" if layer.transposed else "conv_wgrad", layer.R, layer.stride,
                                                              layer.Cin, layer.Cout, a0.N, IH, IW),
                     4 * (sum(p.act.rows * p.act.C for p in pieces) + dy.numel())):
-            _lib.call("dn_conv2d_wgrad", C.byref(d), dy.data_ptr(), dw.data_ptr(), ws.data_ptr(), nbytes, _stream())
+            if bn is not None:
+                by, bnm, dgamma, dbeta = bn
+                _lib.call("dn_conv2d_wgrad_bn_relu", C.byref(d), dy.data_ptr(), by.t.data_ptr(), by.scale.data_ptr(), by.shift.data_ptr(),
+                          by.mean.data_ptr(), by.invstd.data_ptr(), bnm.weight.data_ptr(), dgamma.data_ptr(), dbeta.data_ptr(), by.rows,
+                          dw.data_ptr(), ws.data_ptr(), nbytes, _stream())
+            else:
+                _lib.call("dn_conv2d_wgrad", C.byref(d), dy.data_ptr(), dw.data_ptr(), ws.data_ptr(), nbytes, _stream())
         if sink is not None:
+            if bn is not None:
+                sink.put(bn[1].weight, bn[2])
+                sink.put(bn[1].bias, bn[3])
             sink.put(layer.m.weight, dw)
         return dw
 
@@ -702,6 +728,10 @@
                 cross_stream_use(fresh, main)
         dw = launch()
     cross_stream_use(dy, side)
+    if bn is not None:
+        by, _, dgamma, dbeta = bn
+        for t in (by.t, by.scale, by.shift, by.mean, by.invstd, dgamma, dbeta):
+            cross_stream_use(t, side)
     for p in pieces:
         cross_stream_use(p.act.t, side)
         if p.act.scale is not None:
@@ -880,7 +910,7 @@
         return self.grads.get(id(param))
 
 
-def bn_backward(y, bn, sink, training):
+def bn_backward(y, bn, sink, training, sums_only=False):
     g, y_t, Cn, dev = y.grad, y.t, y.C, y.t.device
     if not training:
         raise NotImplementedError("backward through eval-mode BatchNorm (frozen statistics) is not implemented")
@@ -913,6 +943,11 @@
             dgamma = torch.empty(Cn, dtype=torch.float32, device=dev)
         if dbeta is None:
             dbeta = torch.empty(Cn, dtype=torch.float32, device=dev)
+    if sums_only:
+        if final is None:
+            _lib.call("dn_bn_bwd_sums_finalize", y.partial.data_ptr(), y.partial_rows, y.partial_stride, y.partial_offset, Cn,
+                      dgamma.data_ptr(), dbeta.data_ptr(), _stream())
+        return g, dgamma, dbeta
     if y.pool_src is not None:
         dpooled, pidx = y.pool_src
         hbm_call("dn::bn_bwd_apply_pool_kernel", y.rows * Cn * 8 + y.rows * Cn * 5 // 4, "dn_bn_bwd_apply_pool", dpooled.data_ptr(),
@@ -981,10 +1016,15 @@
     def backward():
         if y.grad is None:
             return
-        g = bn_backward(y, bn, sink, training)
+        fused = training and wgrad_applies_bn(layer, x_piece, y)
+        if fused:
+            g, dgamma, dbeta = bn_backward(y, bn, sink, training, sums_only=True)
+        else:
+            g = bn_backward(y, bn, sink, training)
         if layer.m.bias is not None:
             sink.put_zero(layer.m.bias)
-        conv_wgrad(layer, [x_piece], g, (OH, OW), out=sink.dest(layer.m.weight), sink=sink)
+        conv_wgrad(layer, [x_piece], g, (OH, OW), out=sink.dest(layer.m.weight), sink=sink,
+                   bn=(y, bn, dgamma, dbeta) if fused else None)
         conv_dgrad(layer, g, xa.N, OH, OW, [x_piece], (xa.H, xa.W))
         y.grad = None
 
```

Measured after the change: 2007, median of 6. Within noise of the previous version (+0.7%).
